# utiasSTARS/pyslam

Measured on AMD Instinct MI355X. Metric: ms/LM-iter (Jac build + J^T J + Schur solve), stereo BA @ 500k residuals, lower is better.
Workload: dtype f64

## Files before the change

pyslam_amd/csrc/ps_abi_problem.h:

```cpp


const char* ps_last_error(void) { return g_err.c_str(); }

int ps_device_count(void) {
    int n = 0;
    if (hipGetDeviceCount(&n) != hipSuccess) return 0;
    return n;
}

int ps_warm_up(void) {
    static std::once_flag once;
    static int rc = 0;
    std::call_once(once, [] {
        void* p = nullptr;
        if (hipMalloc(&p, 256) != hipSuccess) { rc = fail("hipMalloc failed (no usable HIP device?)"); return; }
        hipLaunchKernelGGL(k_zero4, dim3(1), dim3(256), 0, 0, (size_t)8, (double*)p, (size_t)0, (double*)nullptr, (size_t)0,
                           (double*)nullptr, (size_t)0, (double*)nullptr);
        double hostw[4] = {0, 0, 0, 0};
        (void)hipMemsetAsync(p, 0, 256, 0);
        (void)hipMemcpyAsync((char*)p + 128, p, 64, hipMemcpyDeviceToDevice, 0);
        (void)hipMemcpyAsync(hostw, p, sizeof(hostw), hipMemcpyDeviceToHost, 0);
        if (hipDeviceSynchronize() != hipSuccess) rc = fail("the warm-up launch failed");
        hipFree(p);
        hipFuncAttributes a;
// ... 769 lines not shown
        } else {
            int32_t init[2] = {0, INT_MAX}, *d_mm = nullptr;
            if (h->alloc(&d_mm, 2, true)) return -1;
            HIP_OK(hipMemcpyAsync(d_mm, init, sizeof(init), hipMemcpyHostToDevice, h->stream));
            hipLaunchKernelGGL(k_lmw_maxobs, dim3(cdiv(nv, 256)), dim3(256), 0, h->stream, nv, h->lm_ptr, d_mm);
            HIP_OK(hipMemcpyAsync(init, d_mm, sizeof(init), hipMemcpyDeviceToHost, h->stream));
            HIP_OK(hipStreamSynchronize(h->stream));
            mx = init[0]; mn = init[1];
        }
        if (mx <= PS_LMW_MAXOBS && mn >= 1) {
            const int W = 64 - (mx - 1), nw = cdiv(Nl, W);
            if (!dev_build) {
                std::vector<int32_t> first((size_t)nw + 1, nv);
                for (int w = 0, v = 0; w < nw; ++w) { while (v < nv && lm_ptr[v] < W * w) ++v; first[w] = v; }
                if (h->upload(&h->lmw_first, first)) return -1;
            } else {
                if (h->alloc(&h->lmw_first, (size_t)nw + 1, true)) return -1;
                hipLaunchKernelGGL(k_lmw_items, dim3(cdiv(nw + 1, 256)), dim3(256), 0, h->stream, nv, nw, W, h->lm_ptr, h->lmw_first);
            }
            h->lmw_nwaves = nw;
            h->nsq_l = std::max(h->nsq_l, cdiv(nw, 4));
        }
    }
    h->nsq_p = nr > 0 ? cdiv(P, 256) : 0;
    if (h->alloc(&h->sq_part_l, (size_t)h->nsq_l) || h->alloc(&h->sq_part_p, (size_t)h->nsq_p) ||
        h->alloc(&h->shard_buf, 2)) return -1;
    if (h->alloc(&h->cost_partials, (size_t)std::max({h->ncost_obs + h->ncost_fac, cdiv(h->lmw_nwaves, 4) + h->ncost_fac, 512}) + 8)) return -1;
    if (h->zero(h->shard_buf, 2 * sizeof(double))) return -1;
    if (!ps_pool().take(ps_pool().host_words, &h->words_host))
        HIP_OK(hipHostMalloc(&h->words_host, PS_WORDS_BYTES, hipHostMallocMapped | hipHostMallocCoherent));
    std::memset(h->words_host, 0, PS_WORDS_BYTES);
    char* wdev = nullptr;
    HIP_OK(hipHostGetDevicePointer((void**)&wdev, h->words_host, 0));
    static_assert(SC_NWORDS * sizeof(double) <= 256 && ST_NWORDS * sizeof(int32_t) <= 256, "result words outgrew their windows");
    char* whost = (char*)h->words_host;
    h->h_scalars = (double*)(whost + 0);      h->h_scalars_dev = (double*)(wdev + 0);
    h->h_status = (int32_t*)(whost + 256);    h->h_status_dev = (int32_t*)(wdev + 256);
    h->h_seq = (long long*)(whost + 512);     h->h_seq_dev = (long long*)(wdev + 512);
    h->h_shard = (double*)(whost + 768);      h->h_shard_dev = (double*)(wdev + 768);
    h->h_setup = (long long*)(whost + 1024);  h->h_setup_dev = (long long*)(wdev + 1024);
    h->h_ldi_fro = (double*)(whost + 1280);   h->h_ldi_fro_dev = (double*)(wdev + 1280);
    h->h_early = (long long*)(whost + 1536);  h->h_early_dev = (long long*)(wdev + 1536);
    h->h_lmfail = (long long*)(whost + 1792); h->h_lmfail_dev = (long long*)(wdev + 1792);
    h->h_mo_hist = (double*)(whost + 2048);   h->h_mo_hist_dev = (double*)(wdev + 2048);
    if (h->alloc(&h->arrivals, 2)) return -1;
    if (h->zero(h->arrivals, 2 * sizeof(int32_t))) return -1;
    if (h->arena_close()) return -1;
    HIP_OK(hipStreamSynchronize(h->stream));
    if (nr >= 16 && nr * D > h->direct_max && h->pcg_variant == 1 && !ps_env("PS_LAZY_COARSE")) {
        if (build_coarse(h)) return -1;
        HIP_OK(hipStreamSynchronize(h->stream));
        lap("two-level structures");
    }
    if (ldi_eligible(h) && h->ldi_direct_ok && h->N == 0 && h->F > 0 && !h->ldi_stream &&
        !ps_pool().take(ps_pool().side_streams, &h->ldi_stream))
        HIP_OK(hipStreamCreateWithFlags(&h->ldi_stream, hipStreamNonBlocking));
    lap("scalars + final sync");
    relook_launch_gates(h);
    guard.ok = true;
    *out = h;
    return 0;
}

int ps_problem_create(const ps_problem_desc* d_in, void* stream, ps_problem** out) {
    return problem_create(d_in, nullptr, stream, out);
}

int ps_problem_create_hybrid(const ps_problem_desc* d_in, const ps_host_rows_desc* rows, void* stream, ps_problem** out) {
    if (!rows) return fail("null argument");
    return problem_create(d_in, rows, stream, out);
}

int ps_set_host_rows(ps_problem* h, const double* rows, int64_t num, double cost) {
    if (!h) return fail("null argument");
    if (!h->hybrid) return fail("ps_set_host_rows: the handle has no host rows (ps_problem_create_hybrid)");
    if (num != h->FH) return fail("ps_set_host_rows: row count differs from the create call's");
    if (num > 0 && !rows) return fail("null argument");
    const size_t FROW = 3 * (size_t)h->D * h->D + 2 * (size_t)h->D;
    if (num > 0) {
        HIP_OK(hipMemcpyAsync(h->fscratch + (size_t)h->F * FROW, rows, (size_t)num * FROW * sizeof(double), hipMemcpyHostToDevice, h->stream));
        HIP_OK(hipStreamSynchronize(h->stream));
    }
    h->host_cost = cost;
    h->prelin_valid = false;
    h->last_cost = h->prev_cost = -1.0;
    return 0;
}
```

pyslam_amd/csrc/ps_abi_solver.h:

```cpp

int ps_get_info(ps_problem* h, ps_problem_info* info) {
    if (!h || !info) return fail("null argument");
    info->dof = h->D; info->num_poses = h->P; info->num_reduced = h->nr; info->num_points = h->L;
    info->num_var_points = h->nv; info->num_obs = h->N; info->num_edges = h->F; info->num_priors = 0;
    info->reduced_nnzb = h->nnzb; info->num_pairs = h->npairs;
    info->reduce_count = ((long)h->nnzb + h->nr) / 2 * h->D * h->D + (long)h->nr * h->D + 3;
    info->device_bytes = (int64_t)h->dev_bytes;
    info->cg_restarts = h->cg_fallbacks;
    info->cg_kernel_launches = h->cg_kernel_launches;
    info->ldi_solves = h->ldi_solves; info->ldi_fallbacks = h->ldi_fallbacks; info->ldi_seeds = h->ldi_seeds;
    info->xcg_fused_solves = h->xf_solves; info->xcg_fused_fallbacks = h->xf_fallbacks;
    info->cg_persist_solves = h->cp_launches; info->cg_persist_failures = h->cp_failures;
    info->cg_persist_refused = h->cp_refused; info->persist_cus = h->persist_cus;
    info->persist_cus_needed = h->cp_ok ? h->cp_cus_needed : (h->xp_ok ? h->xp_cus_needed : 0);
    info->landmark_passes_taken_over = h->prelm_used;
    return 0;
}

int ps_eval_cost(ps_problem* h, int include_all_constant, double* cost) {
    if (!h || !cost) return fail("null argument");
    if (include_all_constant && h->fuse_cost == 1 && lm_cost_possible(h)) { if (lm_cost_pass(h, h->lin_lambda, SC_COST)) return -1; }
    else if (cost_pass(h, include_all_constant, SC_COST)) return -1;
    if (read_scalars(h)) return -1;
    *cost = h->h_scalars[SC_COST];
    if (include_all_constant && !h->hybrid) h->last_cost = *cost;
    return 0;
}

int ps_linearize(ps_problem* h, double lambda) {
    if (!h) return fail("null argument");
    h->last_cost = h->prev_cost = -1.0;
    return linearize(h, lambda);
}

static int ensure_shard_pack(ps_problem* h) {
    if (h->shard_pack) return 0;
    const int nr = h->nr, DD = h->D * h->D;
    std::vector<int32_t> up, upT;
    for (int r = 0; r < nr; ++r)
        for (int b = h->h_row_ptr[r]; b < h->h_row_ptr[r + 1]; ++b) {
            const int c = h->h_col_idx[b];
            if (c < r) continue;
            up.push_back(b);
            const int32_t* lo = h->h_col_idx.data() + h->h_row_ptr[c];
            const int32_t* hi = h->h_col_idx.data() + h->h_row_ptr[c + 1];
            const int32_t* it = std::lower_bound(lo, hi, r);
            if (it == hi || *it != r) return fail("reduced block pattern is not symmetric");
            upT.push_back((int32_t)(it - h->h_col_idx.data()));
        }
    h->nup = (long)up.size();
    h->pack_count = h->nup * DD + (long)nr * h->D + 2 + 1;
    if (h->upload(&h->up_slot, up) || h->upload(&h->upT_slot, upT) || h->alloc(&h->shard_pack, (size_t)h->pack_count)) return -1;
    relook_launch_gates(h);
    return 0;
}

int ps_reduce_buffer(ps_problem* h, void** dev_ptr, int64_t* count) {
    if (!h || !dev_ptr || !count) return fail("null argument");
    if (ensure_shard_pack(h)) return -1;
    *dev_ptr = h->shard_pack; *count = h->pack_count;
    return 0;
}

int ps_shard_pack(ps_problem* h) {
    if (!h) return fail("null argument");
    if (ensure_shard_pack(h)) return -1;
    const long ntail = (long)h->nr * h->D + 2;
    const int nb = (int)std::min<long>(4096, cdiv(h->pack_count, 256));
    if (h->D == 6) hipLaunchKernelGGL(k_shard_pack<6>, dim3(nb), dim3(256), 0, h->stream, h->nup, h->up_slot, h->S, ntail, h->g, h->status, h->shard_pack);
    else hipLaunchKernelGGL(k_shard_pack<3>, dim3(nb), dim3(256), 0, h->stream, h->nup, h->up_slot, h->S, ntail, h->g, h->status, h->shard_pack);
    return 0;
}

int ps_shard_unpack(ps_problem* h) {
    if (!h) return fail("null argument");
    h->prelin_valid = h->prelm_valid = false;
    if (ensure_shard_pack(h)) return -1;
    const long ntail = (long)h->nr * h->D + 2;
    const int nb = (int)std::min<long>(4096, cdiv(h->pack_count, 256));
    if (h->D == 6) hipLaunchKernelGGL(k_shard_unpack<6>, dim3(nb), dim3(256), 0, h->stream, h->nup, h->up_slot, h->upT_slot, h->shard_pack, h->S, ntail, h->g, h->status);
    else hipLaunchKernelGGL(k_shard_unpack<3>, dim3(nb), dim3(256), 0, h->stream, h->nup, h->up_slot, h->upT_slot, h->shard_pack, h->S, ntail, h->g, h->status);
    return 0;
}

static inline double resolve_pcg_tol(const ps_problem* h, double tol) {
    if (tol > 0.0) return tol;
    return h->nv > 0 ? 1e-12 : 1e-14;
}

int ps_solve_reduced(ps_problem* h, double tol, int max_iters, int* iters_out, double* relres_out) {
    if (!h) return fail("null argument");
    tol = resolve_pcg_tol(h, tol);
    const int rc = solve_reduced(h, tol, max_iters, iters_out, relres_out);
    if (rc == 0 && h->h_status[ST_LM_FAIL]) return fail("a landmark block H_ll is not positive definite");
    return rc;
}

static int z_of_last_linearize(ps_problem* h, const char* who) {
    if (!h->z_foreign || h->nv == 0) return 0;
    char buf[320];
    snprintf(buf, sizeof buf, "%s: Z, C^-1 and c no longer belong to the last ps_linearize -- a landmark pass has since run at another point "
             "(ps_eval_cost after the parameters moved, or a whole-iteration call that expected a successor): call ps_linearize again", who);
    return fail(buf);
}

int ps_backsub(ps_problem* h) {
    if (!h) return fail("null argument");
    if (z_of_last_linearize(h, "ps_backsub")) return -1;
    return backsub(h);
}

int ps_get_dx(ps_problem* h, double* dx_pose, double* dx_point) {
    if (!h) return fail("null argument");
    std::vector<double> tmp;
    if (dx_pose && h->nr) HIP_OK(hipMemcpyAsync(dx_pose, h->x, (size_t)h->nr * h->D * sizeof(double), hipMemcpyDefault, h->stream));
    if (dx_point && h->nv) {
        tmp.resize((size_t)h->nv * 3);
        HIP_OK(hipMemcpyAsync(tmp.data(), h->dxl, tmp.size() * sizeof(double), hipMemcpyDeviceToHost, h->stream));
    }
    if (sync(h)) return -1;
    for (int s2 = 0; dx_point && s2 < h->nv; ++s2)
        std::memcpy(dx_point + 3 * (size_t)h->h_vid_of_slot[s2], &tmp[3 * (size_t)s2], 3 * sizeof(double));
    return 0;
}

int ps_step_norm2(ps_problem* h, double* norm2) {
    if (!h || !norm2) return fail("null argument");
    if (step_norm(h) || read_scalars(h)) return -1;
    *norm2 = h->h_scalars[SC_DXP2] + h->h_scalars[SC_DXL2];
    return 0;
}

int ps_apply_update(ps_problem* h, double step) {
    if (!h) return fail("null argument");
    h->prelin_valid = h->prelm_valid = false;
    h->last_cost = h->prev_cost = -1.0;
    return apply_update(h, step);
}

int ps_snapshot_params(ps_problem* h) {
    if (!h) return fail("null argument");
    h->snap_valid = true;
    h->snap_cost = h->last_cost;
    const size_t n1 = (size_t)h->P * h->PW, n2 = (size_t)h->L * 3;
    if (n1 + n2)
        hipLaunchKernelGGL(k_copy2, dim3((unsigned)std::min<size_t>(2048, cdiv((long)(n1 + n2), 256))), dim3(256), 0, h->stream,
                           n1, (const double*)h->poses, h->poses_snap, n2, (const double*)h->points, h->points_snap);
    return 0;
}

static int restore_params_by_exchange(ps_problem* h) {
    if (!h->snap_valid) return fail("ps_solve: no snapshot to restore");
    h->params_moved_since_lin = true;
    h->prelin_valid = h->prelm_valid = false;
    h->last_cost = h->snap_cost; h->prev_cost = -1.0;
    std::swap(h->poses, h->poses_snap);
    std::swap(h->points, h->points_snap);
    h->snap_valid = false;
    return 0;
}

int ps_restore_params(ps_problem* h) {
    if (!h) return fail("null argument");
    if (!h->snap_valid) return fail("ps_restore_params: no snapshot (none taken, or ps_solve has consumed it)");
    h->params_moved_since_lin = true;
    h->prelin_valid = h->prelm_valid = false;
    h->last_cost = h->snap_cost; h->prev_cost = -1.0;
    const size_t n1 = (size_t)h->P * h->PW, n2 = (size_t)h->L * 3;
    if (n1 + n2)
        hipLaunchKernelGGL(k_copy2, dim3((unsigned)std::min<size_t>(2048, cdiv((long)(n1 + n2), 256))), dim3(256), 0, h->stream,
                           n1, (const double*)h->poses_snap, h->poses, n2, (const double*)h->points_snap, h->points);
    return 0;
}

int ps_get_params(ps_problem* h, double* poses, double* points) {
    if (!h) return fail("null argument");
    if (poses && h->P) HIP_OK(hipMemcpyAsync(poses, h->poses, (size_t)h->P * h->PW * sizeof(double), hipMemcpyDefault, h->stream));
    if (points && h->L) HIP_OK(hipMemcpyAsync(points, h->points, (size_t)h->L * 3 * sizeof(double), hipMemcpyDefault, h->stream));
    return sync(h);
}

int ps_set_params(ps_problem* h, const double* poses, const double* points) {
    if (!h) return fail("null argument");
    h->params_moved_since_lin = true;
    h->prelin_valid = h->prelm_valid = false;
    h->last_cost = h->prev_cost = -1.0;
    if (poses && h->P) HIP_OK(hipMemcpyAsync(h->poses, poses, (size_t)h->P * h->PW * sizeof(double), hipMemcpyDefault, h->stream));
    if (points && h->L) HIP_OK(hipMemcpyAsync(h->points, points, (size_t)h->L * 3 * sizeof(double), hipMemcpyDefault, h->stream));
    return sync(h);
}

int ps_gn_finish(ps_problem* h, int linesearch, double* cost_out, double* dx_pose_norm2, double* dx_point_norm2) {
    if (!h) return fail("null argument");
    if (z_of_last_linearize(h, "ps_gn_finish")) return -1;
    HIP_OK(hipMemsetAsync(h->scalars + SC_DXP2, 0, sizeof(double), h->stream));
    HIP_OK(hipMemsetAsync(h->scalars + SC_DXL2, 0, sizeof(double), h->stream));
    if (gn_tail(h, linesearch, nullptr)) return -1;
    if (read_scalars(h)) return -1;
    if (h->h_status[ST_LM_FAIL]) return fail("a landmark block H_ll is not positive definite");
    if (cost_out) *cost_out = linesearch ? h->h_scalars[SC_COST] : h->h_scalars[SC_LINCOST];
    if (dx_pose_norm2) *dx_pose_norm2 = h->h_scalars[SC_DXP2];
    if (dx_point_norm2) *dx_point_norm2 = h->h_scalars[SC_DXL2];
    return 0;
}

int ps_gn_solve_finish(ps_problem* h, double pcg_tol, int pcg_max_iters, int linesearch, double* cost_out,
                       double* dx_pose_norm2, double* dx_point_norm2, int* pcg_iters_out, double* pcg_relres_out) {
    if (!h) return fail("null argument");
    pcg_tol = resolve_pcg_tol(h, pcg_tol);
    if (z_of_last_linearize(h, "ps_gn_solve_finish")) return -1;
    HIP_OK(hipMemsetAsync(h->scalars + SC_DXP2, 0, sizeof(double), h->stream));
    HIP_OK(hipMemsetAsync(h->scalars + SC_DXL2, 0, sizeof(double), h->stream));
    if (h->nr > 0 && h->pcg_variant == 1) {
        const int rc = h->D == 6
            ? gn_solve_and_finish_async<6>(h, pcg_tol, pcg_max_iters, linesearch, pcg_iters_out, pcg_relres_out, nullptr)
            : gn_solve_and_finish_async<3>(h, pcg_tol, pcg_max_iters, linesearch, pcg_iters_out, pcg_relres_out, nullptr);
        if (rc) return -1;
    } else {
        if (solve_reduced(h, pcg_tol, pcg_max_iters, pcg_iters_out, pcg_relres_out)) return -1;
        if (gn_tail(h, linesearch, nullptr)) return -1;
        if (read_scalars(h)) return -1;
    }
    if (h->h_status[ST_LM_FAIL]) return fail("a landmark block H_ll is not positive definite");
    if (cost_out) *cost_out = linesearch ? h->h_scalars[SC_COST] : h->h_scalars[SC_LINCOST];
    if (dx_pose_norm2) *dx_pose_norm2 = h->h_scalars[SC_DXP2];
    if (dx_point_norm2) *dx_point_norm2 = h->h_scalars[SC_DXL2];
    return 0;
}

int ps_set_segment_exchange(ps_problem* h, void* nccl_all_gather_fn, int32_t world, int32_t rank, int64_t maxlen,
                            int64_t n_mine, const int64_t* mine, int64_t n_dst, const int64_t* dst, const int64_t* src_ptr,
                            const int64_t* src_off) {
    if (!h) return fail("null argument");
    if (!nccl_all_gather_fn) { h->seg_allgather = nullptr; return 0; }
    if (!(h->nccl_allreduce && h->nccl_comm)) return fail("ps_set_segment_exchange: call ps_set_collective first");
    if (ensure_shard_pack(h)) return -1;
    const int64_t T = 3, body = h->pack_count - T;
    if (world < 1 || rank < 0 || rank >= world || n_mine < 0 || n_dst < 0 || maxlen < T + n_mine || (n_mine && !mine) ||
        (n_dst && (!dst || !src_ptr || !src_off)))
        return fail("ps_set_segment_exchange: inconsistent plan");
    for (int64_t k = 0; k < n_mine; ++k) if (mine[k] < 0 || mine[k] >= body) return fail("ps_set_segment_exchange: an element of this rank lies outside [upper(S) | g]");
    for (int64_t k = 0; k < n_dst; ++k) {
        if (dst[k] < 0 || dst[k] >= body || src_ptr[k + 1] < src_ptr[k]) return fail("ps_set_segment_exchange: bad destination table");
        for (int64_t q = src_ptr[k]; q < src_ptr[k + 1]; ++q) {
            const int64_t r = src_off[q] / maxlen, o = src_off[q] % maxlen;
            if (src_off[q] < 0 || r >= world || o < T || (q > src_ptr[k] && src_off[q] / maxlen <= src_off[q - 1] / maxlen))
                return fail("ps_set_segment_exchange: bad source table (offsets must be rank * maxlen + 3 + k, ascending rank)");
        }
    }
    if (n_dst && src_ptr[0] != 0) return fail("ps_set_segment_exchange: src_ptr must start at 0");
    if ((int64_t)world * maxlen > INT32_MAX || body > INT32_MAX) return fail("ps_set_segment_exchange: the exchange does not fit 32-bit plan entries");
    const std::vector<int32_t> vm(mine, mine + n_mine), vd(dst, dst + n_dst), vp(src_ptr, src_ptr + (n_dst ? n_dst + 1 : 0)),
                               vo(src_off, src_off + (n_dst ? src_ptr[n_dst] : 0));
    if (h->upload(&h->seg_mine, vm) || h->upload(&h->seg_dst, vd) || h->upload(&h->seg_src_ptr, vp) || h->upload(&h->seg_src_off, vo) ||
        h->alloc(&h->seg_in, (size_t)maxlen) || h->alloc(&h->seg_all, (size_t)maxlen * world)) return -1;
    h->seg_world = world; h->seg_maxlen = maxlen; h->seg_nmine = n_mine; h->seg_ndst = n_dst;
    h->seg_allgather = (ps_problem::allgather_fn)nccl_all_gather_fn;
    return 0;
}

static int exchange_reduced_system(ps_problem* h) {
    enum { NCCL_F64 = 8, NCCL_SUM = 0 };
    if (!h->seg_allgather) {
        { StageTimer tpk(h, PS_ST_PACK); if (ps_shard_pack(h)) return -1; }
        {
            StageTimer tar(h, PS_ST_ALLREDUCE);
            if (h->nccl_allreduce(h->shard_pack, h->shard_pack, (size_t)h->pack_count, NCCL_F64, NCCL_SUM, h->nccl_comm, h->stream))
                return fail("ncclAllReduce of the reduced system failed");
        }
        { StageTimer tpk(h, PS_ST_PACK); if (ps_shard_unpack(h)) return -1; }
        return 0;
    }
    h->prelin_valid = h->prelm_valid = false;
    const long T = 3, ntail = (long)h->nr * h->D + 2;
    const unsigned nb1 = (unsigned)std::min<long>(2048, cdiv(h->seg_maxlen, 256)), nb2 = (unsigned)std::min<long>(4096, cdiv(h->seg_ndst + T, 256));
    {
        StageTimer tpk(h, PS_ST_PACK);
        if (h->D == 6) hipLaunchKernelGGL(k_seg_pack<6>, dim3(nb1), dim3(256), 0, h->stream, h->nup, h->up_slot, h->S, ntail, h->g, h->status, T, h->seg_nmine, h->seg_mine, h->seg_in, h->seg_maxlen);
        else hipLaunchKernelGGL(k_seg_pack<3>, dim3(nb1), dim3(256), 0, h->stream, h->nup, h->up_slot, h->S, ntail, h->g, h->status, T, h->seg_nmine, h->seg_mine, h->seg_in, h->seg_maxlen);
    }
    {
        StageTimer tar(h, PS_ST_ALLREDUCE);
        if (h->seg_allgather(h->seg_in, h->seg_all, (size_t)h->seg_maxlen, NCCL_F64, h->nccl_comm, h->stream))
            return fail("ncclAllGather of the reduced system's segments failed");
    }
    {
        StageTimer tpk(h, PS_ST_PACK);
        if (h->D == 6) hipLaunchKernelGGL(k_seg_sum<6>, dim3(nb2), dim3(256), 0, h->stream, h->seg_ndst, h->seg_dst, h->seg_src_ptr, h->seg_src_off, h->seg_all, T, h->seg_world, h->seg_maxlen, h->nup, h->up_slot, h->upT_slot, h->S, ntail, h->g, h->status);
        else hipLaunchKernelGGL(k_seg_sum<3>, dim3(nb2), dim3(256), 0, h->stream, h->seg_ndst, h->seg_dst, h->seg_src_ptr, h->seg_src_off, h->seg_all, T, h->seg_world, h->seg_maxlen, h->nup, h->up_slot, h->upT_slot, h->S, ntail, h->g, h->status);
    }
    return 0;
}

int ps_set_collective(ps_problem* h, void* nccl_all_reduce_fn, void* nccl_comm) {
    if (!h) return fail("null argument");
    if (h->hybrid && nccl_comm) return fail("a hybrid handle (host rows) is not landmark-sharded");
    h->nccl_allreduce = (ps_problem::allreduce_fn)nccl_all_reduce_fn;
    h->nccl_comm = nccl_comm;
    relook_launch_gates(h);
    return 0;
}

int ps_shard_buffer(ps_problem* h, void** dev_ptr) {
    if (!h || !dev_ptr) return fail("null argument");
    *dev_ptr = h->shard_buf;
    return 0;
}

int ps_gn_solve_finish_enqueue(ps_problem* h, double pcg_tol, int pcg_max_iters, int linesearch, int first) {
    if (!h) return fail("null argument");
    if (h->nr == 0 || h->pcg_variant != 1) return fail("ps_gn_solve_finish_enqueue needs the fused CG and a reduced system");
    pcg_tol = resolve_pcg_tol(h, pcg_tol);
    if (first && z_of_last_linearize(h, "ps_gn_solve_finish_enqueue")) return -1;
    h->shard_out = true;
    h->no_repeat = !(h->nccl_allreduce && h->nccl_comm);
    struct Reset { ps_problem* h; ~Reset() { h->shard_out = false; h->no_repeat = false; } } reset{h};
    if (first) {
        HIP_OK(hipMemsetAsync(h->scalars + SC_DXP2, 0, sizeof(double), h->stream));
        if (!h->coarse_built && build_coarse(h)) return -1;
        if (!(h->nccl_allreduce && h->nccl_comm) && h->xf_skip == 0) h->xf_skip = 1;
        if (h->cg_explicit) { if (h->D == 6 ? xcg_setup<6>(h, pcg_max_iters, true) : xcg_setup<3>(h, pcg_max_iters, true)) return -1; }
        else if (h->D == 6 ? cg_fused_setup<6>(h, pcg_max_iters, true) : cg_fused_setup<3>(h, pcg_max_iters, true)) return -1;
    }
    const int limit = pcg_max_iters + (h->cg_explicit ? 1 : 2);
    const bool big_step = h->prev_cost > 0.0 && h->last_cost > 0.0 && std::fabs(h->prev_cost - h->last_cost) > 0.05 * h->prev_cost;
    const int margin = big_step ? (h->cg_explicit ? 5 : std::max(6, h->cg_margin))
                                : ((h->cg_explicit || h->last_pcg_iters == h->prev_pcg_iters) ? std::min(2, h->cg_margin) : h->cg_margin);
    int count = first ? (h->last_pcg_iters > 0 ? h->last_pcg_iters + margin : (h->cg_explicit ? 32 : 24)) : std::max(8, h->cg_launched / 2);
    count = std::min(count, limit - h->cg_launched);
    const bool last = count <= 0;
    const int32_t* gate = last ? nullptr : h->status;
    if (h->cg_explicit) {
        if (!last) {
            const int head = std::min(count, 12);
            if (h->D == 6) { xcg_launch<6>(h, pcg_tol, head); if (xcg_side_enqueue<6>(h)) return -1; xcg_launch<6>(h, pcg_tol, count - head); }
            else { xcg_launch<3>(h, pcg_tol, head); if (xcg_side_enqueue<3>(h)) return -1; xcg_launch<3>(h, pcg_tol, count - head); }
        }
        if (h->D == 6) hipLaunchKernelGGL(k_cg_unscale<6>, dim3(cdiv((long)h->nr * 6, 256)), dim3(256), 0, h->stream, h->nr, h->Linv, h->cg_xh, h->x, gate);
        else hipLaunchKernelGGL(k_cg_unscale<3>, dim3(cdiv((long)h->nr * 3, 256)), dim3(256), 0, h->stream, h->nr, h->Linv, h->cg_xh, h->x, gate);
    } else if (h->D == 6) { if (!last) cg_fused_launch<6>(h, pcg_tol, count); cg_fused_recover<6>(h, gate); }
    else { if (!last) cg_fused_launch<3>(h, pcg_tol, count); cg_fused_recover<3>(h, gate); }
    if (gn_tail(h, linesearch, last ? nullptr : h->status)) return -1;
    return last ? 1 : 0;
}

int ps_gn_result(ps_problem* h, int* done, double* shard2 , double* dx_pose_norm2,
                 int* pcg_iters_out, double* pcg_relres_out) {
    if (!h) return fail("null argument");
    double sb[2] = {0.0, 0.0};
    HIP_OK(hipMemcpyAsync(sb, h->shard_buf, sizeof(sb), hipMemcpyDeviceToHost, h->stream));
    if (read_scalars(h)) return -1;
    if (h->h_status[ST_LM_FAIL]) return fail("a landmark block H_ll is not positive definite");
    if (done) *done = h->h_status[ST_PCG_DONE];
    if (shard2) { shard2[0] = sb[0]; shard2[1] = sb[1]; }
    if (dx_pose_norm2) *dx_pose_norm2 = h->h_scalars[SC_DXP2];
    if (h->h_status[ST_PCG_DONE]) { h->prev_cost = h->last_cost; h->last_cost = sb[0]; }
// ... 195 lines not shown

static int lm_iteration_impl(ps_problem* h, double lambda, double pcg_tol, int pcg_max_iters, int linesearch, double* cost_out,
                             double* dx_norm_out, double* model_decrease_out, int* pcg_iters_out, double* pcg_relres_out,
                             double* start_cost_out) {
    if (!h) return fail("null argument");
    if (h->nccl_allreduce && h->nccl_comm) return fail("ps_lm_iteration: not offered for a landmark-sharded handle");
    if (!linesearch) return fail("ps_lm_iteration: the gain ratio needs the cost AFTER the step (linesearch != 0)");
    if (!(lambda >= 0.0) || !std::isfinite(lambda)) return fail("ps_lm_iteration: lambda must be finite and >= 0");
    const int expect_was = h->expect_next;
    const bool spec_was = h->spec_next;
    h->expect_next = 0; h->spec_next = false;
    h->lm_md = true;
    const int rc = gn_iteration_impl(h, lambda, pcg_tol, pcg_max_iters, linesearch, cost_out, dx_norm_out, pcg_iters_out, pcg_relres_out,
                                     start_cost_out);
    h->lm_md = false;
    h->expect_next = expect_was; h->spec_next = spec_was;
    if (rc) return rc;
    if (model_decrease_out) *model_decrease_out = h->h_scalars[SC_MODELDEC];
    return 0;
}

int ps_lm_iteration(ps_problem* h, double lambda, double pcg_tol, int pcg_max_iters, int linesearch, double* cost_out,
                    double* dx_norm_out, double* model_decrease_out, int* pcg_iters_out, double* pcg_relres_out) {
    return lm_iteration_impl(h, lambda, pcg_tol, pcg_max_iters, linesearch, cost_out, dx_norm_out, model_decrease_out, pcg_iters_out,
                             pcg_relres_out, nullptr);
}

int ps_solve_lm(ps_problem* h, const ps_lm_options* o, double pcg_tol, int pcg_max_iters, double* cost_history, int32_t cap,
                int32_t* n_history, int32_t* iterations, double* last_dx_norm, int32_t* pcg_iters, double* pcg_relres, double* iter_ms,
                double* lm_rows) {
    if (!h || !o || !cost_history || !n_history) return fail("null argument");
    if (h->nccl_allreduce && h->nccl_comm) return 1;
    if (h->hybrid) return 1;
    if (o->max_iters < 0 || (long)o->max_iters + 2 > cap) return 1;
    if (!(o->lambda_min > 0.0) || !(o->lambda_max >= o->lambda_min)) return fail("ps_solve_lm: 0 < lambda_min <= lambda_max expected");
    if (ps_reset_solver_state(h)) return -1;
    auto clamp = [&](double v) { return std::min(std::max(v, o->lambda_min), o->lambda_max); };
    double lam = clamp(o->lambda0 > 0.0 ? o->lambda0 : 1e-3), nu = 2.0;
    int n = 0, it = 0;
    double cost = 0.0, dxn = 0.0;
    bool done = false;
    while (!done) {
        ++it;
        h->solve_horizon = -1;
        if (ps_snapshot_params(h)) return -1;
        const auto t0 = std::chrono::steady_clock::now();
        double c0 = 0.0, c = 0.0, rel = 0.0, md = 0.0;
        int its = 0;
        if (lm_iteration_impl(h, lam, pcg_tol, pcg_max_iters, o->linesearch, &c, &dxn, &md, &its, &rel, it == 1 ? &c0 : nullptr)) return -1;
        if (it == 1) { cost = c0; cost_history[n++] = c0; }
        const double prev = cost;
        const bool ok = std::isfinite(md) && md > 0.0 && std::isfinite(c);
        const double rho = ok ? (prev - c) / md : -1.0;
        const double used = lam, raw = lam * nu;
        const bool accepted = rho > 0.0;
        if (accepted) {
            const double q = 2.0 * rho - 1.0;
            cost = c; lam = clamp(lam * std::max(1.0 / 3.0, 1.0 - q * q * q)); nu = 2.0;
        } else {
            lam = clamp(raw); nu *= 2.0;
            if (restore_params_by_exchange(h)) return -1;
            h->last_cost = prev;
        }
        if (lm_rows) { double* r = lm_rows + 4 * (size_t)(it - 1); r[0] = used; r[1] = rho; r[2] = accepted ? 1.0 : 0.0; r[3] = md; }
        if (pcg_iters) pcg_iters[it - 1] = its;
        if (pcg_relres) pcg_relres[it - 1] = rel;
        if (iter_ms) iter_ms[it - 1] = std::chrono::duration<double, std::milli>(std::chrono::steady_clock::now() - t0).count();
        cost_history[n++] = cost;
        static_assert(offsetof(ps_lm_options, lambda0) == sizeof(ps_solve_options), "ps_lm_options begins with ps_solve_options' fields");
        done = ps_stop_base(reinterpret_cast<const ps_solve_options*>(o), it, cost, dxn);
        if (accepted) done = done || cost >= o->min_cost_decrease * prev;
        else done = done || raw > o->lambda_max;
    }
    h->snap_valid = false;
    *n_history = n;
    if (iterations) *iterations = it;
    if (last_dx_norm) *last_dx_norm = dxn;
    return 0;
}

int ps_motion_only_solve(ps_problem* h, const ps_solve_options* o, double* cost_history, int32_t cap, int32_t* n_history,
                         int32_t* iterations, double* last_dx_norm, double* pose12_out) {
    if (!h || !o || !cost_history || !n_history) return fail("null argument");
    h->prelin_valid = h->prelm_valid = false;
    const bool eligible = h->mo_fused && !h->hybrid && h->nv == 0 && h->F == 0 && h->nr == 1 && h->P == 1 && h->D == 6 && h->N == h->Np &&
                          h->pcg_variant == 1 && h->max_pose_obs <= 2048;
    const int need = o->max_iters + 2;
    if (!eligible || need + 16 > PS_MO_HIST_WORDS || need > cap) return 1;
    h->cov_ready = false;
    h->last_cost = h->prev_cost = -1.0;
    if (!h->status_clean) {
        HIP_OK(hipMemsetAsync(h->status, 0, ST_NWORDS * sizeof(int32_t), h->stream));
        h->status_clean = true;
    }
    const ObsWide wp{h->sidx_p, h->stiff_tab};
    const long long seq_now = ++h->seq;
    StageTimer total(h, PS_ST_TOTAL, 2);
    if (h->wide_obs)
        hipLaunchKernelGGL(k_motion_only_solve<true>, dim3(1), dim3(PS_MO_THREADS), 0, h->stream, h->pitems, h->pitem_ptr, h->pobs,
                           h->points, h->ogroups, h->poses, *o, h->x, h->status, h->scalars, h->h_mo_hist_dev, PS_MO_HIST_WORDS,
                           h->h_status_dev, h->h_scalars_dev, h->h_seq_dev, seq_now, wp);
    else
        hipLaunchKernelGGL(k_motion_only_solve<false>, dim3(1), dim3(PS_MO_THREADS), 0, h->stream, h->pitems, h->pitem_ptr, h->pobs,
                           h->points, h->ogroups, h->poses, *o, h->x, h->status, h->scalars, h->h_mo_hist_dev, PS_MO_HIST_WORDS,
                           h->h_status_dev, h->h_scalars_dev, h->h_seq_dev, seq_now, wp);
    total.stop();
    if (wait_published(h)) return -1;
    if (h->h_status[ST_DIAG_FAIL]) {
        h->status_clean = false;
        return fail("reduced system has a non-positive-definite diagonal block (gauge freedom? hold a pose constant or add a prior)");
    }
    const int n = (int)h->h_mo_hist[0];
    if (n < 1 || n > cap) return fail("ps_motion_only_solve: cost history out of range");
    for (int k = 0; k < n; ++k) cost_history[k] = h->h_mo_hist[15 + k];
    if (pose12_out) for (int k = 0; k < 12; ++k) pose12_out[k] = h->h_mo_hist[3 + k];
    *n_history = n;
    if (iterations) *iterations = (int32_t)h->h_mo_hist[1];
    if (last_dx_norm) *last_dx_norm = h->h_mo_hist[2];
    h->last_cost = cost_history[n - 1];
    return 0;
}

int ps_covariance_begin(ps_problem* h) {
    if (!h) return fail("null argument");
    cov_release(h);
    ++h->cov_epoch;
    h->prelin_valid = h->prelm_valid = false;
    if (linearize(h, 0.0)) return -1;
    if (h->nr > 0 && h->pcg_variant == 1 && !use_direct(h) && !h->coarse_built && build_coarse(h)) return -1;
    if (h->nr > 0 && h->pcg_variant == 1 && !use_direct(h) && !h->cg_explicit) {
        const int rc = h->D == 6 ? cg_fused_setup<6>(h, 16) : cg_fused_setup<3>(h, 16);
        if (rc) return -1;
    }
    if (read_scalars(h)) return -1;
    if (h->h_status[ST_LM_FAIL]) return fail("a landmark block H_ll is not positive definite");
    if (h->h_status[ST_DIAG_FAIL]) return fail("reduced system has a non-positive-definite diagonal block (gauge freedom? hold a pose constant or add a prior)");
    if (h->h_slot_of_vid.size() != h->h_vid_of_slot.size()) {
        h->h_slot_of_vid.assign(h->h_vid_of_slot.size(), 0);
        for (size_t s2 = 0; s2 < h->h_vid_of_slot.size(); ++s2) h->h_slot_of_vid[h->h_vid_of_slot[s2]] = (int32_t)s2;
    }
    h->cov_ready = true;
    return 0;
}

int ps_covariance_column(ps_problem* h, int kind, int index, int comp, double tol, int max_iters,
                         int* iters_out, double* relres_out) {
    if (!h) return fail("null argument");
    tol = resolve_pcg_tol(h, tol);
    if (!h->cov_ready) return fail("ps_covariance_column: call ps_covariance_begin first (any linearisation invalidates it)");
    if (kind == 0 ? (index < 0 || index >= h->nr || comp < 0 || comp >= h->D)
                  : (kind != 1 || index < 0 || index >= h->nv || comp < 0 || comp >= 3))
        return fail("ps_covariance_column: parameter index / component out of range");
    if (h->nr) HIP_OK(hipMemsetAsync(h->g, 0, (size_t)h->nr * h->D * sizeof(double), h->stream));
    if (h->nv) HIP_OK(hipMemsetAsync(h->cvec, 0, (size_t)h->nv * 3 * sizeof(double), h->stream));
    const int slot = kind == 1 ? h->h_slot_of_vid[index] : index;
    hipLaunchKernelGGL(k_cov_rhs, dim3(1), dim3(64), 0, h->stream, kind, slot, comp, h->D, h->lm_ptr, h->lobs,
                       h->pose_rid, h->Z, h->Cinv, h->g, h->cvec);
    int its = 0; double rel = 0.0;
    if (h->nr > 0) {
        int rc;
        if (use_direct(h)) {
            rc = h->D == 6 ? direct_solve_enqueue<6>(h) : direct_solve_enqueue<3>(h);
            if (!rc) rc = read_scalars(h);
            if (!rc) rc = cg_report(h, &its, &rel);
        } else if (h->pcg_variant == 1 && h->cg_explicit)
            rc = h->D == 6 ? xcg_run<6>(h, tol, max_iters, &its, &rel) : xcg_run<3>(h, tol, max_iters, &its, &rel);
        else if (h->pcg_variant == 1)
            rc = h->D == 6 ? cg_fused_run<6>(h, tol, max_iters, &its, &rel, true) : cg_fused_run<3>(h, tol, max_iters, &its, &rel, true);
        else
            rc = h->D == 6 ? pcg_run<6>(h, tol, max_iters, &its, &rel) : pcg_run<3>(h, tol, max_iters, &its, &rel);
        if (rc) return -1;
    }
    if (backsub(h)) return -1;
    if (iters_out) *iters_out = its;
    if (relres_out) *relres_out = rel;
    return 0;
}

int ps_get_reduced_system(ps_problem* h, int32_t* row_ptr, int32_t* col_idx, double* vals, double* g) {
    if (!h) return fail("null argument");
    if (row_ptr) std::memcpy(row_ptr, h->h_row_ptr.data(), h->h_row_ptr.size() * sizeof(int32_t));
    if (col_idx) std::memcpy(col_idx, h->h_col_idx.data(), h->h_col_idx.size() * sizeof(int32_t));
    if (vals && h->nnzb) HIP_OK(hipMemcpyAsync(vals, h->S, (size_t)h->nnzb * h->D * h->D * sizeof(double), hipMemcpyDeviceToHost, h->stream));
    if (g && h->nr) HIP_OK(hipMemcpyAsync(g, h->g, (size_t)h->nr * h->D * sizeof(double), hipMemcpyDeviceToHost, h->stream));
    return sync(h);
}

int ps_get_landmark_factors(ps_problem* h, double* cinv, double* c) {
    if (!h) return fail("null argument");
    if (z_of_last_linearize(h, "ps_get_landmark_factors")) return -1;
    std::vector<double> t6((size_t)h->nv * 6), t3((size_t)h->nv * 3);
    if (h->nv) {
        HIP_OK(hipMemcpyAsync(t6.data(), h->Cinv, t6.size() * sizeof(double), hipMemcpyDeviceToHost, h->stream));
        HIP_OK(hipMemcpyAsync(t3.data(), h->cvec, t3.size() * sizeof(double), hipMemcpyDeviceToHost, h->stream));
    }
    if (sync(h)) return -1;
    for (int s2 = 0; s2 < h->nv; ++s2) {
        const size_t v = (size_t)h->h_vid_of_slot[s2];
        if (cinv) std::memcpy(cinv + 6 * v, &t6[6 * (size_t)s2], 6 * sizeof(double));
        if (c) std::memcpy(c + 3 * v, &t3[3 * (size_t)s2], 3 * sizeof(double));
    }
    return 0;
}

int ps_debug_reproj_blocks(ps_problem* h, double* r, double* jpose, double* jpoint) {
    if (!h || !r || !jpose || !jpoint) return fail("null argument");
    if (h->N == 0) return 0;
    double *dr, *djp, *djl;
    HIP_OK(hipMalloc((void**)&dr, (size_t)h->N * 3 * sizeof(double)));
    HIP_OK(hipMalloc((void**)&djp, (size_t)h->N * 18 * sizeof(double)));
    HIP_OK(hipMalloc((void**)&djl, (size_t)h->N * 9 * sizeof(double)));
    const ObsWide wl{h->sidx_l, h->stiff_tab};
    if (h->wide_obs)
        hipLaunchKernelGGL(k_debug_reproj<true>, dim3(cdiv(h->N, 256)), dim3(256), 0, h->stream, h->N, h->lobs, h->lorig,
                       h->poses, h->points, h->ogroups, dr, djp, djl, wl);
    else
        hipLaunchKernelGGL(k_debug_reproj<false>, dim3(cdiv(h->N, 256)), dim3(256), 0, h->stream, h->N, h->lobs, h->lorig,
                       h->poses, h->points, h->ogroups, dr, djp, djl, wl);
    hipMemcpyAsync(r, dr, (size_t)h->N * 3 * sizeof(double), hipMemcpyDeviceToHost, h->stream);
    hipMemcpyAsync(jpose, djp, (size_t)h->N * 18 * sizeof(double), hipMemcpyDeviceToHost, h->stream);
    hipMemcpyAsync(jpoint, djl, (size_t)h->N * 9 * sizeof(double), hipMemcpyDeviceToHost, h->stream);
    const int rc = sync(h);
    hipFree(dr); hipFree(djp); hipFree(djl);
    return rc;
}

int ps_debug_factor_blocks(ps_problem* h, double* r, double* j1, double* j2) {
    if (!h || !r || !j1 || !j2) return fail("null argument");
    if (h->F == 0) return 0;
    const int D = h->D, DD = D * D, ROW = D + 2 * DD;
    double* dbg;
    HIP_OK(hipMalloc((void**)&dbg, (size_t)h->F * ROW * sizeof(double)));
    const int rc0 = D == 6 ? launch_factor_pass<6>(h, 0.0, dbg) : launch_factor_pass<3>(h, 0.0, dbg);
    std::vector<double> t((size_t)h->F * ROW);
    hipMemcpyAsync(t.data(), dbg, t.size() * sizeof(double), hipMemcpyDeviceToHost, h->stream);
    const int rc = sync(h);
    hipFree(dbg);
    if (rc0 || rc) return -1;
    for (long f = 0; f < h->F; ++f) {
        std::memcpy(r + f * D, &t[(size_t)f * ROW], D * sizeof(double));
        std::memcpy(j1 + f * DD, &t[(size_t)f * ROW + D], DD * sizeof(double));
        std::memcpy(j2 + f * DD, &t[(size_t)f * ROW + D + DD], DD * sizeof(double));
    }
    return 0;
}

int ps_debug_table_checksums(ps_problem* h, uint64_t* out, int capacity, int* count) {
    if (!h || !out || !count) return fail("null argument");
    if (sync(h)) return -1;
    struct Tab { const void* p; size_t bytes; };
    const bool tiled = h->schur_tiles > 1 && h->npair_items > 0;
    const Tab tabs[16] = {
        {h->point_vid, (size_t)h->L * 4}, {h->lobs, (size_t)h->N * sizeof(LObs)}, {h->lorig, (size_t)h->N * 4},
        {h->lm_ptr, ((size_t)h->nv + 1) * 4}, {h->lm_point, (size_t)h->nv * 4}, {h->pose_of_rid, (size_t)std::max(h->nr, 1) * 4},
        {h->pitems, (size_t)h->npitems * sizeof(PItem)}, {h->pitem_ptr, ((size_t)h->nr + 1) * 4}, {h->pobs, (size_t)h->Np * sizeof(LObs)},
        {h->pairs, (size_t)h->npairs * 8}, {h->pair_xitems, (size_t)8 * h->pair_per_xcd * sizeof(PairItem)},
        {tiled ? h->comb_items : nullptr, (size_t)h->ncomb * sizeof(PairItem)}, {tiled ? h->comb_tasks : nullptr, (size_t)h->npair_items * 4},
        {h->row_ptr, ((size_t)h->nr + 1) * 4}, {h->col_idx, (size_t)h->nnzb * 4}, {h->diag_slot, (size_t)h->nr * 4}};
    *count = 16;
    std::vector<unsigned char> buf;
    for (int t = 0; t < 16 && t < capacity; ++t) {
        uint64_t hsh = 0;
        if (tabs[t].p && tabs[t].bytes) {
            buf.resize(tabs[t].bytes);
            HIP_OK(hipMemcpy(buf.data(), tabs[t].p, tabs[t].bytes, hipMemcpyDeviceToHost));
            hsh = 1469598103934665603ull;
            size_t i = 0;
            for (; i + 8 <= buf.size(); i += 8) { uint64_t w; std::memcpy(&w, &buf[i], 8); hsh = (hsh ^ w) * 1099511628211ull; }
            for (; i < buf.size(); ++i) hsh = (hsh ^ buf[i]) * 1099511628211ull;
        }
        out[t] = hsh;
    }
    return 0;
}

static void relook_path(ps_problem* h) {
    const bool possible = ps_ldi_possible(*h, (long)h->nr * h->D);
    if (h->coarse_built && possible != h->xmin_auto_ldi && h->cg_explicit_min_rows < 0) h->coarse_built = false;
}

int ps_set_option(ps_problem* h, const char* name, double value) {
    if (!h || !name) return fail("null argument");
    if (!std::strcmp(name, "expect_next")) { h->expect_next = value != 0 && !h->hybrid; return 0; }
    if (!std::strcmp(name, "solve_horizon")) { h->solve_horizon = value < 0 ? -1 : (int)std::min(value, 1e6); return 0; }
    h->prelin_valid = h->prelm_valid = false;
    const char* refusal = nullptr;
    const int fx = ps_option_apply(*h, name, value, &refusal);
    if (fx == PS_OPT_UNKNOWN) return fail(std::string("unknown option: ") + name);
    if (fx == PS_OPT_REFUSED) return fail(refusal);
    if (fx & PS_FX_COARSE_REBUILD) h->coarse_built = false;
    if (fx & PS_FX_DROP_FACTOR) h->lci_next = -1;
    if (fx & PS_FX_DROP_SIDE) h->side_todo = false;
    if ((fx & PS_FX_LDI_OFF) && !h->ldi_enable) { h->ldi_cur = -1; if (h->ldi_state != 1) h->ldi_state = 0; }
    if (fx & PS_FX_RELOOK_PATH) relook_path(h);
    relook_launch_gates(h);
    return 0;
}

int ps_get_option(ps_problem* h, const char* name, double* value) {
    if (!h || !name || !value) return fail("null argument");
    const std::string n(name);
    if (n == "lin_zero_list") *value = h->lin_zero_gate ? 1.0 : 0.0;
    else if (n == "lin_fills") *value = (double)h->lin_fills;
    else if (n == "lin_zero_launches") *value = (double)h->lin_zero_launches;
    else return fail("ps_get_option: no read-back for option: " + n);
    return 0;
}

int ps_reset_solver_state(ps_problem* h) {
    if (!h) return fail("null argument");
    h->prelin_valid = h->prelm_valid = false;
    if (!h->solver_touched) {
        static_cast<PsCostHistory&>(*h) = PsCostHistory{};
        return 0;
    }
    h->solver_touched = false;
    HIP_OK(hipStreamSynchronize(h->stream));
    if (h->side) HIP_OK(hipStreamSynchronize(h->side));
    if (h->ldi_stream) HIP_OK(hipStreamSynchronize(h->ldi_stream));
    drain_timers(h);
    static_cast<PsCarried&>(*h) = PsCarried{};
    static_cast<PsCostHistory&>(*h) = PsCostHistory{};
    if (h->lag_status) HIP_OK(hipMemsetAsync(h->lag_status, 0, ST_NWORDS * sizeof(int32_t), h->stream));
    if (h->ldi_ready && !(h->ldi_direct_ok && h->N == 0 && h->F > 0)) h->ldi_direct = false;
    h->cov_ready = false;
    return 0;
}

#ifndef PS_BUILD_SHA
#define PS_BUILD_SHA "unknown"
#endif
const char* ps_build_sha(void) { return PS_BUILD_SHA; }

int ps_set_profiling(ps_problem* h, int enabled) {
    if (!h) return fail("null argument");
    h->profiling = enabled < 0 ? 0 : (enabled > 2 ? 2 : enabled);
    return 0;
}

int ps_get_stage_times(ps_problem* h, double* ms, int64_t* counts, int reset) {
    if (!h) return fail("null argument");
    if (!h->pending.empty() && sync(h)) return -1;
    for (int i = 0; i < PS_NUM_STAGES; ++i) {
        if (ms) ms[i] = h->stage_ms[i];
        if (counts) counts[i] = h->stage_n[i];
        if (reset) { h->stage_ms[i] = 0.0; h->stage_n[i] = 0; }
    }
    return 0;
}

int ps_dense_normal_solve(const double* J, const double* r, int32_t m, int32_t n, double* dx, double* covariance) {
    if (!J || !r || !dx || m <= 0 || n <= 0) return fail("bad argument");
    if (n > 2048) return fail("generic (host-evaluated) path supports at most 2048 unknowns");
    int ndev = 0;
    if (hipGetDeviceCount(&ndev) != hipSuccess || ndev == 0) return fail("no HIP device visible");
    const int nrhs = covariance ? n + 1 : 1;
    DevBuf bJ, br, bH, bB, bst, bg;
    if (bJ.get((size_t)m * n * sizeof(double)) || br.get((size_t)m * sizeof(double)) || bH.get((size_t)n * n * sizeof(double)) ||
        bB.get((size_t)n * nrhs * sizeof(double)) || bst.get(ST_NWORDS * sizeof(int32_t)) || bg.get((size_t)n * sizeof(double))) return -1;
    double *dJ = bJ.as<double>(), *dr = br.as<double>(), *dH = bH.as<double>(), *dB = bB.as<double>(), *dg = bg.as<double>();
    int32_t* dst = bst.as<int32_t>();
    HIP_OK(hipMemset(dst, 0, ST_NWORDS * sizeof(int32_t)));
    HIP_OK(hipMemcpy(dJ, J, (size_t)m * n * sizeof(double), hipMemcpyHostToDevice));
    HIP_OK(hipMemcpy(dr, r, (size_t)m * sizeof(double), hipMemcpyHostToDevice));
    hipLaunchKernelGGL(k_dense_normal, dim3(cdiv((long)n * n, 256)), dim3(256), 0, 0, m, n, dJ, dr, dH, dg);
    std::vector<double> B((size_t)n * nrhs, 0.0), gh(n);
    HIP_OK(hipMemcpy(gh.data(), dg, (size_t)n * sizeof(double), hipMemcpyDeviceToHost));
    for (int i = 0; i < n; ++i) { B[(size_t)i * nrhs] = gh[i]; if (covariance) B[(size_t)i * nrhs + 1 + i] = 1.0; }
    HIP_OK(hipMemcpy(dB, B.data(), B.size() * sizeof(double), hipMemcpyHostToDevice));
    hipLaunchKernelGGL(k_dense_chol_solve, dim3(1), dim3(256), 0, 0, n, nrhs, dH, dB, dst);
    HIP_OK(hipMemcpy(B.data(), dB, B.size() * sizeof(double), hipMemcpyDeviceToHost));
    int32_t st[ST_NWORDS];
    HIP_OK(hipMemcpy(st, dst, sizeof(st), hipMemcpyDeviceToHost));
    for (int i = 0; i < n; ++i) {
        dx[i] = B[(size_t)i * nrhs];
        if (covariance) for (int j = 0; j < n; ++j) covariance[(size_t)i * n + j] = B[(size_t)i * nrhs + 1 + j];
    }
    if (st[ST_DIAG_FAIL]) return fail("normal matrix is not positive definite");
    return 0;
}
```

pyslam_amd/csrc/ps_abi_triang.h:

```cpp

int ps_triangulate(ps_problem* h, int64_t n, const int32_t* vids, int refine_iters, double min_parallax_deg, int write_back,
                   double* points_out, int32_t* status_out) {
    if (!h) return fail("null argument");
    if (h->nv > 0 && h->D != 6) return fail("ps_triangulate: landmarks on a problem whose poses are not SE(3)");
    if (refine_iters < 0 || refine_iters > 1000) return fail("ps_triangulate: refine_iters must lie in [0, 1000]");
    if (!(min_parallax_deg >= 0.0 && min_parallax_deg <= 180.0)) return fail("ps_triangulate: min_parallax_deg must lie in [0, 180]");
    if (!vids) n = h->nv;
    if (n < 0) return fail("ps_triangulate: negative count");
    if (n == 0) return 0;
    if (n >= (1L << 31) / 16) return fail("ps_triangulate: too many landmarks for one call");
    if (h->h_slot_of_vid.size() != h->h_vid_of_slot.size()) {
        h->h_slot_of_vid.assign(h->h_vid_of_slot.size(), 0);
        for (size_t s2 = 0; s2 < h->h_vid_of_slot.size(); ++s2) h->h_slot_of_vid[h->h_vid_of_slot[s2]] = (int32_t)s2;
    }
    std::vector<int32_t> slots;
    if (vids) {
        slots.resize((size_t)n);
        for (int64_t k = 0; k < n; ++k) {
            if (vids[k] < 0 || vids[k] >= h->nv)
                return fail("ps_triangulate: landmark index " + std::to_string(vids[k]) + " out of range (variable landmarks: " +
                            std::to_string(h->nv) + ")");
            slots[k] = h->h_slot_of_vid[vids[k]];
        }
    }
    const size_t words = (size_t)n * 3 + (size_t)n;
    if (h->tri_cap < words) {
        if (h->tri_buf) { hipStreamSynchronize(h->stream); hipFree(h->tri_buf); h->tri_buf = nullptr; h->tri_cap = 0; }
        void* p = nullptr;
        const hipError_t e = hipMalloc(&p, words * sizeof(double));
        if (e != hipSuccess) return fail(std::string("ps_triangulate: hipMalloc: ") + hipGetErrorString(e));
        h->tri_buf = (double*)p; h->tri_cap = words;
    }
    double* d_pts = h->tri_buf;
    int32_t* d_status = reinterpret_cast<int32_t*>(h->tri_buf + (size_t)n * 3);
    int32_t* d_slots = d_status + n;
    hipStream_t st = h->stream;
    if (vids) HIP_OK(hipMemcpyAsync(d_slots, slots.data(), (size_t)n * sizeof(int32_t), hipMemcpyHostToDevice, st));
    const double cos_min = std::cos(min_parallax_deg * (3.14159265358979323846 / 180.0));
    const ObsWide wl{h->sidx_l, h->stiff_tab};
    const dim3 grid(cdiv(n, 256 / PS_LM_GROUP)), block(256);
    if (h->wide_obs)
        hipLaunchKernelGGL(k_triangulate<true>, grid, block, 0, st, (int)n, vids ? d_slots : (const int32_t*)nullptr, h->lm_ptr, h->lm_point,
                           h->lobs, h->poses, h->points, h->ogroups, wl, refine_iters, cos_min, write_back ? 1 : 0, d_pts, d_status);
    else
        hipLaunchKernelGGL(k_triangulate<false>, grid, block, 0, st, (int)n, vids ? d_slots : (const int32_t*)nullptr, h->lm_ptr, h->lm_point,
                           h->lobs, h->poses, h->points, h->ogroups, wl, refine_iters, cos_min, write_back ? 1 : 0, d_pts, d_status);
    if (write_back) {
        h->params_moved_since_lin = true;
        h->prelin_valid = h->prelm_valid = false;
        h->last_cost = h->prev_cost = -1.0;
    }
    std::vector<double> pts(points_out && !vids ? (size_t)n * 3 : 0);
    std::vector<int32_t> stat(status_out && !vids ? (size_t)n : 0);
    if (points_out) HIP_OK(hipMemcpyAsync(vids ? points_out : pts.data(), d_pts, (size_t)n * 3 * sizeof(double), hipMemcpyDeviceToHost, st));
    if (status_out) HIP_OK(hipMemcpyAsync(vids ? status_out : stat.data(), d_status, (size_t)n * sizeof(int32_t), hipMemcpyDeviceToHost, st));
    if (sync(h)) return -1;
    if (!vids)
        for (int64_t s2 = 0; s2 < n; ++s2) {
            const int32_t vid = h->h_vid_of_slot[s2];
            if (points_out) std::memcpy(points_out + 3 * (size_t)vid, &pts[3 * (size_t)s2], 3 * sizeof(double));
            if (status_out) status_out[vid] = stat[s2];
        }
    return 0;
}
```

pyslam_amd/csrc/ps_core.hip:

```cpp
#include <hip/hip_runtime.h>

#include <algorithm>
#include <array>
#include <map>
#include <atomic>
#include <chrono>
#include <thread>
#include <climits>
#include <cmath>
#include <cstdio>
#include <cstring>
#include <memory>
#include <mutex>
#include <string>
#include <vector>

#include "pyslam_hip.h"
#include "ps_kernels.h"
#include "ps_ransac.h"
#include "ps_k_twoview.h"
#include "ps_k_pnp.h"
#include "ps_photo.h"
#include "ps_k_dense.h"
#include "ps_k_feat.h"
// ... 120 lines not shown
    double xcg_tag_lambda[2] = {0.0, 0.0}, xcg_setup_lambda = 0.0;
    bool mc_active = false;
    bool last_setup_lagx = false;
    int xf_skip = 0;
    int ldi_state = 0;
    int ldi_cur = -1, ldi_next = -1;
    long ldi_iter = 0, ldi_ready_at = 0;
    bool ldi_side_todo = false, ldi_update_ok = false, ldi_sread_pending = false;
    int ldi_last_its = 0, ldi_prev_its = 0;
    int ldi_rejects = 0; long ldi_no_seed_before = 0;
    double ldi_tag = -1.0, ldi_next_tag = -1.0, ldi_call_start_cost = -1.0;
    double ldi_prev_start_cost = -2.0;
    bool ldi_moved = false;
    int last_pcg_iters = 0;
    int prev_pcg_iters = -1;
};

struct ps_problem : PsOptions, PsCostHistory, PsCarried {
    hipStream_t stream = nullptr;
    bool own_stream = false;
    int D = 6, PW = 12;
    int P = 0, nr = 0, L = 0, nv = 0;
    long N = 0, Nl = 0, Np = 0;
    long F = 0;
    long FH = 0;
    bool hybrid = false;
    double host_cost = 0.0;
    long npairs = 0;
    int nnzb = 0;
    size_t dev_bytes = 0;
    std::vector<void*> allocs;
    struct Guard { char* guard; size_t table_bytes; int serial; };
    std::vector<Guard> guards;
    int check_guards(const char* where) {
        int bad = 0;
        std::vector<unsigned char> g(4096);
        for (const Guard& gd : guards) {
            if (hipMemcpy(g.data(), gd.guard, 4096, hipMemcpyDeviceToHost) != hipSuccess) return -1;
            for (int i = 0; i < 4096; ++i) if (g[i] != 0xA5) {
                fprintf(stderr, "GUARD %p %s: table #%d (%zu bytes) overrun at +%d (byte %02x)\n", (void*)this, where, gd.serial, gd.table_bytes, i, g[i]);
                ++bad; break;
            }
        }
        return bad;
    }

    double *poses = nullptr, *points = nullptr, *poses_snap = nullptr, *points_snap = nullptr;
    int32_t *pose_rid = nullptr, *point_vid = nullptr;
    ObsGroup* ogroups = nullptr;
    bool wide_obs = false;
    int32_t *sidx_l = nullptr, *sidx_p = nullptr;
    double* stiff_tab = nullptr;
    LObs* lobs = nullptr;
    int32_t *lorig = nullptr, *lm_ptr = nullptr, *lm_point = nullptr;
    double *Z = nullptr, *Cinv = nullptr, *cvec = nullptr, *dxl = nullptr;
    LObs* pobs = nullptr;
    PItem* pitems = nullptr;
    int npitems = 0;
    int32_t* pitem_ptr = nullptr;
    double* ppartial = nullptr;
    int2* pairs = nullptr;
    int npair_items = 0, pair_per_xcd = 0;
    PairItem* pair_xitems = nullptr;
    int schur_tiles = 1, ncomb = 0;
    bool has_diag_tasks = false;
    double* Spart = nullptr;
    PairItem* comb_items = nullptr;
    int32_t* comb_tasks = nullptr;
    FactorGroup* fgroups = nullptr;
    int32_t *f_i = nullptr, *f_j = nullptr, *f_grp = nullptr;
    double *f_Tinv = nullptr, *fscratch = nullptr;
    int32_t *eslots = nullptr, *eptr = nullptr, *eslot_diag = nullptr, *gptr = nullptr, *gitems = nullptr;
    int2* eitems = nullptr;
    int nes = 0;
    int32_t *row_ptr = nullptr, *col_idx = nullptr, *diag_slot = nullptr;
    double* red = nullptr;
    long red_count = 0;
    double *S = nullptr, *g = nullptr;
    int32_t* zero_slots = nullptr;
    int nzero_slots = 0;
    bool has_extra_pairs = false;
    bool lin_zero_gate = false;
    long lin_fills = 0, lin_zero_launches = 0;
    std::vector<int32_t> h_row_ptr, h_col_idx;
    std::vector<int32_t> h_vid_of_slot;
    double *x = nullptr, *r = nullptr, *z = nullptr, *p0 = nullptr, *p1 = nullptr, *q = nullptr, *Minv = nullptr;
    double *rz_part = nullptr, *rr_part = nullptr, *pq_part = nullptr, *hist = nullptr;
    int npartA = 0, npartB = 0, hist_cap = 0;
    double *Linv = nullptr, *cg_r[2] = {}, *cg_w[2] = {}, *cg_s[2] = {}, *cg_gd[2] = {}, *cg_xh = nullptr;
    int32_t* brow_of = nullptr;
    double* cg_p = nullptr;
    double* Saug = nullptr;
    int32_t* ident_slot = nullptr;
    int G = 0, ncb = 0, nc = 0, nr_aug = 0, nnzb_aug = 0;
    size_t cg_cap = 0, saug_cap = 0;
    int32_t *pnode = nullptr, *slo = nullptr, *shi = nullptr, *run_lo = nullptr, *run_hi = nullptr,
            *arow_ptr = nullptr, *acol_idx = nullptr, *aug_slot = nullptr, *fine_nnz = nullptr;
    double *pw0 = nullptr, *pw1 = nullptr, *SZ = nullptr, *Ac = nullptr, *tvec = nullptr, *chol_scratch = nullptr;
    double *Bmat = nullptr, *bgv = nullptr, *SB = nullptr, *BSZ = nullptr;
    double *Bmat2[2] = {}, *X2[2] = {}, *Mpart = nullptr;
    bool lagx_ok = false;
    int side_buf = 0;
    double host_wait_ns = 0.0, host_call_ns = 0.0;
    long host_waits = 0, host_calls = 0;
    size_t rows_lds = 0;
    bool rows_attr_set = false, rows_lci_lds = false;
    int32_t *ent_ptr = nullptr, *ent_q = nullptr, *ent_lo = nullptr, *ent_hi = nullptr;
    int32_t *seg_ptr = nullptr, *seg_ent = nullptr, *seg_row = nullptr;
    int max_row_ents = 0;
    int32_t* pose_of_rid = nullptr;
    double *Lci2[2] = {}, *LciT2[2] = {};
    hipStream_t side = nullptr;
    int side_cus = 0;
    hipEvent_t ev_ac = nullptr, ev_chol = nullptr, ev_acdone = nullptr;
    unsigned long long* chk_sums = nullptr; int chk_nsum = 0;
    double *chk_Ac = nullptr, *chk_BSZ = nullptr, *chk_Ac_side = nullptr; int32_t* chk_cnt = nullptr; size_t chk_bsz_n = 0;
    int32_t* lag_status = nullptr;
    double* Mc = nullptr;
    bool coarse_built = false;
    bool coarse_clamped = false;
    int max_pose_obs = 0;
    double* mo_partials = nullptr;
    bool status_clean = true;
    double *dA = nullptr, *dLi = nullptr, *dLiT = nullptr;
    bool cg_explicit = false;
    double lin_lambda = 0.0;
    double *xstate = nullptr, *xy = nullptr, *xp2 = nullptr;
    int ac_bw = -1;
    std::unique_ptr<BandPart> bpart;
    double *Lrow = nullptr, *Lcol = nullptr, *rdiag = nullptr;
    bool xcg_rt_ok = false;
    int xcg_rt_rows = PS_XCG_ROWS_RT;
    int32_t *xcg_wg_out = nullptr, *xcg_nptr = nullptr;
    double *tq_part = nullptr, *tvec2 = nullptr;
    bool xf_ok = false, xf_active = false;
    bool xf_one_ok = false, xf_two = false;
    int32_t *xf_cptr = nullptr, *xf_cols = nullptr, *xf_nlo = nullptr, *xf_nhi = nullptr, *xf_rec = nullptr;
    uint16_t* xf_lidx = nullptr;
    double *xf_tq[2] = {}, *xf_ts[2] = {}, *xf_t[2] = {};
    int xf_rmax = 1, xf_nwg = 0, xf_pf = 2;
    size_t xf_nrec = 0;
    long xf_solves = 0, xf_fallbacks = 0;
    bool cp_ok = false;
    bool cp_recovered = false;
    int cp_ntasks = 0, cg_max_launches = 0;
    void* cp_tasks = nullptr;
    int32_t* cp_row_task0 = nullptr;
    unsigned long long* cp_exch = nullptr;
    unsigned cp_salt = 0;
    long cp_launches = 0, cp_failures = 0;
    int persist_dev = 0, persist_cus = 0;
    bool persist_masked = false;
    int cp_cus_needed = 0, xp_cus_needed = 0;
    int persist_held = 0;
    bool params_moved_since_lin = false;
    bool z_foreign = false;
    bool no_repeat = false;
    long cp_refused = 0;
    void persist_release() { if (persist_held) { ps_persist_ledger().release(persist_dev, persist_held); persist_held = 0; } }
    int persist_capacity() const { return persist_masked ? persist_cus / 2 : persist_cus; }
    bool persist_reserve(int need) {
        if (need <= 0 || persist_cus <= 0) return false;
        if (persist_held) return true;
        if (!ps_persist_ledger().reserve(persist_dev, need, persist_capacity())) { ++cp_refused; return false; }
        persist_held = need; return true;
    }
// ... 127 lines not shown
        dev_bytes += bytes;
        *out = (T*)p;
        return 0;
    }
    char* slab = nullptr; size_t slab_left = 0;
    int slab_reserve(size_t bytes) {
        if (ps_env("PS_ALLOC_GUARD")) return 0;
        void* p = nullptr;
        hipError_t e = hipMalloc(&p, bytes);
        if (e != hipSuccess) return fail(std::string("hipMalloc: ") + hipGetErrorString(e));
        if (ps_env("PS_ARENA_POISON") && hipMemset(p, 0xFF, bytes) != hipSuccess) return fail("hipMemset (poison) failed");
        allocs.push_back(p);
        slab = (char*)p; slab_left = bytes;
        return 0;
    }
    void slab_close() { slab = nullptr; slab_left = 0; }
    bool in_arena(const void* p) const {
        return arena_open && (const char*)p >= arena_dev && (const char*)p < arena_dev + PS_ARENA_BYTES;
    }
    template <typename T>
    int upload(T** out, const T* src, size_t n, bool src_resident = false) {
        if (alloc(out, n)) return -1;
        if (!n) return 0;
        if (src_resident) {
            if (in_arena(*out)) HIP_OK(hipMemcpy(arena_host + ((char*)*out - arena_dev), src, n * sizeof(T), hipMemcpyDeviceToHost));
            else HIP_OK(hipMemcpy(*out, src, n * sizeof(T), hipMemcpyDeviceToDevice));
            return 0;
        }
        if (in_arena(*out)) std::memcpy(arena_host + ((char*)*out - arena_dev), src, n * sizeof(T));
        else HIP_OK(hipMemcpy(*out, src, n * sizeof(T), hipMemcpyHostToDevice));
        return 0;
    }
    template <typename T>
    int upload(T** out, const std::vector<T>& v) { return upload(out, v.data(), v.size()); }
    int zero(void* p, size_t bytes) {
        if (in_arena(p)) return 0;
        HIP_OK(hipMemsetAsync(p, 0, std::max<size_t>(bytes, 1), stream));
        return 0;
    }
    int arena_begin() {
        PsPool& pool = ps_pool();
        void *d = nullptr, *m = nullptr;
        if (!pool.take(pool.dev_arenas, &d)) HIP_OK(hipMalloc(&d, PS_ARENA_BYTES));
        arena_dev = (char*)d;
        if (!pool.take(pool.host_arenas, &m)) HIP_OK(hipHostMalloc(&m, PS_ARENA_BYTES, hipHostMallocDefault));
        arena_host = (char*)m;
        static const bool poison = ps_env("PS_ARENA_POISON") != nullptr;
        if (poison) std::memset(arena_host, 0xFF, PS_ARENA_BYTES);
        arena_poisoned = poison;
        arena_used = 0;
        arena_open = true;
        return 0;
    }
    int arena_flush() {
        if (arena_open && arena_used) HIP_OK(hipMemcpyAsync(arena_dev, arena_host, arena_used, hipMemcpyHostToDevice, stream));
        return 0;
    }
    int arena_close() {
        arena_open = false;
        if (arena_poisoned) arena_used = PS_ARENA_BYTES;
        if (arena_used) HIP_OK(hipMemcpyAsync(arena_dev, arena_host, arena_used, hipMemcpyHostToDevice, stream));
        return 0;
    }
    void arena_release() {
        PsPool& pool = ps_pool();
        if (arena_dev && !pool.give(pool.dev_arenas, (void*)arena_dev)) hipFree(arena_dev);
        if (arena_host && !pool.give(pool.host_arenas, (void*)arena_host)) hipHostFree(arena_host);
        if (words_host && !pool.give(pool.host_words, words_host)) hipHostFree(words_host);
        arena_dev = arena_host = nullptr; words_host = nullptr;
    }
};

inline void cov_release(ps_problem* h) {
    if (!h->cov_buf) return;
    hipStreamSynchronize(h->stream);
    hipFree(h->cov_buf);
    h->cov_buf = nullptr;
    h->cov_sigma_epoch = -1;
}

inline void relook_launch_gates(ps_problem* h) {
    const bool shard = (h->nccl_allreduce && h->nccl_comm) || h->seg_allgather || h->shard_pack || h->has_extra_pairs;
    h->lin_zero_gate = h->lin_zero_list && h->zero_slots && !h->Spart && h->schur_pipeline && h->npitems > 0 && h->D == 6 && !shard;
}

#include "ps_host_cg.h"
#include "ps_host_ldi.h"
#include "ps_host_iteration.h"
#include "ps_host_build.h"

extern "C" {

#include "ps_abi_problem.h"
#include "ps_abi_solver.h"
#include "ps_abi_cov.h"
#include "ps_abi_triang.h"
#include "ps_abi_small.h"
#include "ps_abi_twoview.h"
#include "ps_abi_pnp.h"
#include "ps_abi_dense.h"
#include "ps_abi_feat.h"

}
```

pyslam_amd/csrc/ps_host_cg.h:

```cpp

namespace {

struct StageTimer {
    ps_problem* h;
    int stage;
    hipEvent_t a = nullptr, b = nullptr;
    int slot = -1;
    StageTimer(ps_problem* h_, int st, int level = 2) : h(h_), stage(st) {
        if (h->profiling < level) return;
        if (h->profiling == 1 && h->prof_every > 1 &&
            h->prof_tick % h->prof_every != (st == PS_ST_CG_KERNEL ? h->prof_every / 2 : 0)) return;
        if (h->ev_used + 2 > h->ev_pool.size()) {
            for (int i = 0; i < 64; ++i) { hipEvent_t e; hipEventCreate(&e); h->ev_pool.push_back(e); }
        }
        slot = (int)h->ev_used;
        a = h->ev_pool[h->ev_used++];
        b = h->ev_pool[h->ev_used++];
        hipEventRecord(a, h->stream);
    }
    void stop() {
        if (!a) return;
        hipEventRecord(b, h->stream);
        h->pending.push_back({stage, slot});
        a = nullptr;
    }
    ~StageTimer() { stop(); }
};

void drain_timers(ps_problem* h) {
    for (auto& pr : h->pending) {
        float ms = 0.f;
        if (hipEventElapsedTime(&ms, h->ev_pool[pr.second], h->ev_pool[pr.second + 1]) == hipSuccess) {
            h->stage_ms[pr.first] += ms;
            h->stage_n[pr.first] += 1;
        }
    }
    h->pending.clear();
    h->ev_used = 0;
}

int side_kick(ps_problem* h);
int ldi_side_kick(ps_problem* h);
int linearize(ps_problem* h, double lambda, bool allow_prelm = false);

void drain_timers_ready(ps_problem* h) {
    std::vector<std::pair<int, int>> keep;
    for (auto& pr : h->pending) {
        float ms = 0.f;
        if (hipEventQuery(h->ev_pool[pr.second + 1]) != hipSuccess) { keep.push_back(pr); continue; }
        if (hipEventElapsedTime(&ms, h->ev_pool[pr.second], h->ev_pool[pr.second + 1]) == hipSuccess) {
            h->stage_ms[pr.first] += ms;
            h->stage_n[pr.first] += 1;
        }
    }
    h->pending.swap(keep);
    if (h->pending.empty()) h->ev_used = 0;
}

int sync(ps_problem* h) {
    HIP_OK(hipStreamSynchronize(h->stream));
    h->persist_release();
    drain_timers(h);
    if (h->side_todo) h->side_ready = true;
    return 0;
}

int wait_published(ps_problem* h) {
    volatile long long* w = h->h_seq;
    struct WaitClock {
        ps_problem* h; std::chrono::steady_clock::time_point t0 = std::chrono::steady_clock::now();
        ~WaitClock() { h->host_wait_ns += std::chrono::duration<double, std::nano>(std::chrono::steady_clock::now() - t0).count(); ++h->host_waits; }
    } wc{h};
    static const int kick_mode = ps_env("PS_SIDE_KICK") ? atoi(ps_env("PS_SIDE_KICK")) : 2;
    volatile long long* ws = h->h_setup;
    for (long spins = 0; spins < 400000000L; ++spins) {
        if (kick_mode == 2 && h->side_todo && !h->side_ready && *ws == h->setup_seq) { h->side_ready = true; if (side_kick(h)) return -1; }
        if (h->ldi_side_todo && *ws == h->setup_seq) { if (ldi_side_kick(h)) return -1; }
        if (h->early_armed && *reinterpret_cast<volatile long long*>(h->h_early) == h->early_seq) {
            h->early_armed = false; h->spec_enqueued = true;
            if (h->prelm_pending) { h->prelm_pending = false; h->prelm_valid = true; }
            if (linearize(h, h->lin_lambda, true)) return -1;
        }
        if (*w == h->seq) {
            h->persist_release();
            if (h->lmfail_check && *reinterpret_cast<volatile long long*>(h->h_lmfail + (h->lmfail_check & 1)) == h->lmfail_check) h->h_status[ST_LM_FAIL] += 1;
            if (h->h_status[ST_PERSIST_FAIL] && (h->cg_persist || h->xcg_persist)) { h->cg_persist = 0; h->xcg_persist = 0; ++h->cp_failures; }
            if (h->start_cost_pending) {
                h->start_cost_pending = false;
                h->last_cost = h->ldi_call_start_cost = h->h_scalars[SC_STARTCOST];
            }
            if (h->side_todo) { h->side_ready = true; if (kick_mode >= 1 && side_kick(h)) return -1; }
            if (h->ldi_side_todo) { if (h->spec_enqueued) h->ldi_side_todo = false; else if (ldi_side_kick(h)) return -1; }
            h->early_armed = false;
            if (h->pending.empty()) return 0;
            if (h->spec_enqueued) { drain_timers_ready(h); return 0; }
            HIP_OK(hipEventSynchronize(h->ev_pool[h->pending.back().second + 1]));
            drain_timers(h);
            return 0;
        }
        __builtin_ia32_pause();
    }
    return sync(h);
}

int read_scalars(ps_problem* h) {
    HIP_OK(hipMemcpyAsync(h->h_scalars, h->scalars, SC_NWORDS * sizeof(double), hipMemcpyDeviceToHost, h->stream));
    HIP_OK(hipMemcpyAsync(h->h_status, h->status, ST_NWORDS * sizeof(int32_t), hipMemcpyDeviceToHost, h->stream));
    return sync(h);
}

struct PairRec { uint64_t key; int32_t a, b, tile; };

template <int D>
int launch_factor_pass(ps_problem* h, double lambda, double* dbg = nullptr) {
    if (h->F == 0 && h->FH == 0) return 0;
    if (h->F > 0)
        hipLaunchKernelGGL(k_factor_pass<D>, dim3(cdiv(h->F, PS_FP_FACTORS)), dim3(256), 0, h->stream, (int)h->F, h->f_i,
                           h->f_j, h->f_Tinv, h->f_grp, h->fgroups, h->poses, h->fscratch, dbg);
    if (dbg) return 0;
    const long threads = (long)h->nes * D * D + (long)h->nr * D;
    hipLaunchKernelGGL(k_factor_assemble<D>, dim3(cdiv(threads, 256)), dim3(256), 0, h->stream, h->nes,
                       h->eslots, h->eptr, h->eitems, h->eslot_diag, h->nr, h->gptr, h->gitems,
                       h->fscratch, lambda, h->S, h->g);
    return 0;
}

// ... 383 lines not shown
inline void copy_doubles(hipStream_t st, double* dst, const double* src, size_t n) {
    if (!n) return;
    hipLaunchKernelGGL(k_copy2, dim3((unsigned)std::min<size_t>(2048, cdiv((long)n, 256))), dim3(256), 0, st, n, src, dst, (size_t)0,
                       (const double*)nullptr, (double*)nullptr);
}

template <int D>
int coarse_factor(ps_problem* h, hipStream_t st, int buf, int32_t* stat) {
    const int nc = h->nc, ncb = h->ncb;
    if (nc <= 90) {
        const size_t chol_lds = 2 * (size_t)nc * nc * sizeof(double);
        if (ensure_dynamic_lds((const void*)k_coarse_chol<D, true>, (size_t)(chol_lds))) return -1;
        hipLaunchKernelGGL((k_coarse_chol<D, true>), dim3(1), dim3(1024), chol_lds, st, ncb, h->Ac, h->Lci2[buf],
                           h->LciT2[buf], stat, nullptr);
    } else if (h->big_chol) {
        double* A = h->chol_scratch;
        double* Tinv = A + (size_t)nc * nc;
        copy_doubles(st, A, h->Ac, (size_t)nc * nc);
        const int nsteps = cdiv(nc, PS_BC_W);
        for (int s2 = 0; s2 < nsteps; ++s2) {
            const int j0 = s2 * PS_BC_W, w = std::min(PS_BC_W, nc - j0), m = nc - j0 - w;
            hipLaunchKernelGGL(k_bchol_panel, dim3(std::max(1, cdiv((long)m * w, 1024))), dim3(256), 0, st, nc, j0, A,
                               Tinv + (size_t)s2 * PS_BC_W * PS_BC_W, stat);
            if (m > 0) {
                const int nt = cdiv(m, 32);
                hipLaunchKernelGGL(k_bchol_update, dim3(nt * (nt + 1) / 2), dim3(256), 0, st, nc, j0, w, A);
            }
        }
        const bool dense_out = nc > PS_BI_S0 && !h->cg_explicit;
        if (dense_out) {
            HIP_OK(hipMemsetAsync(h->Lci2[buf], 0, (size_t)nc * nc * sizeof(double), st));
            HIP_OK(hipMemsetAsync(h->LciT2[buf], 0, (size_t)nc * nc * sizeof(double), st));
        }
        const size_t inv_lds = ((size_t)PS_BI_S0 + PS_BC_W) * PS_BI_CW * sizeof(double);
        hipLaunchKernelGGL(k_btri_inverse, dim3(cdiv(nc, PS_BI_CW)), dim3(256), inv_lds, st, nc, A, Tinv, h->Lci2[buf], h->LciT2[buf]);
        for (int s2 = PS_BI_S0; s2 < nc; s2 *= 2) {
            const int pairs = cdiv(nc, 2 * s2), nt = cdiv(s2, PS_BM_T);
            for (int stage = 0; stage < 2; ++stage)
                hipLaunchKernelGGL(k_btri_merge, dim3(pairs * nt * nt), dim3(256), 0, st, nc, s2, stage, A, h->Lci2[buf], h->LciT2[buf]);
        }
        if (dense_out)
            hipLaunchKernelGGL(k_btri_clear, dim3(cdiv((long)nc * nc, 256)), dim3(256), 0, st, nc, h->LciT2[buf]);
    } else {
        hipLaunchKernelGGL((k_coarse_chol<D, false>), dim3(1), dim3(1024), 0, st, ncb, h->Ac, h->Lci2[buf],
                           h->LciT2[buf], stat, h->chol_scratch);
    }
    return 0;
}

template <int D>
int xcg_coarse_inverse(ps_problem* h, hipStream_t st, int buf, int32_t* stat) {
    const int nc = h->nc;
    if (h->band_chol && h->ac_bw >= 0 && h->band_part) {
        const int B = std::max(h->ac_bw, 1), m = h->band_part_m > 0 ? h->band_part_m : BandPart::auto_m(h->ncb, B);
        if (BandPart::eligible(h->ncb, B, m)) {
            if (!h->bpart || h->bpart->ncb != h->ncb || h->bpart->B != B || h->bpart->m != m || h->bpart->D != D) {
                if (h->bpart) { HIP_OK(hipStreamSynchronize(st)); if (h->side) HIP_OK(hipStreamSynchronize(h->side)); h->dev_bytes -= h->bpart->bytes; }
                h->bpart.reset(new BandPart());
                if (h->bpart->build(h->ncb, D, B, m, st)) { h->bpart.reset(); return -1; }
                h->dev_bytes += h->bpart->bytes;
            }
            return h->bpart->run<D>(st, h->Ac, nc, (float*)h->LciT2[buf], nc, stat);
        }
    }
    if (h->band_chol && h->ac_bw >= 0) {
        HIP_OK(hipMemsetAsync(h->Lrow, 0, (size_t)nc * PS_BAND_W * sizeof(double), st));
        HIP_OK(hipMemsetAsync(h->Lcol, 0, (size_t)nc * PS_BAND_W * sizeof(double), st));
        hipLaunchKernelGGL(k_band_chol<D>, dim3(1), dim3(256), 0, st, h->ncb, std::max(h->ac_bw, 1), (const double*)h->Ac, h->Lrow, h->Lcol, h->rdiag, stat,
                           nc, (const int2*)nullptr);
        static const bool inv_dot = ps_env("PS_BAND_INV_DOT") != nullptr;
        if (inv_dot)
            hipLaunchKernelGGL(k_band_inverse, dim3(cdiv(nc, 4)), dim3(256), 0, st, nc, h->Lrow, h->Lcol, h->rdiag,
                               h->chol_scratch, (float*)h->LciT2[buf]);
        else
            hipLaunchKernelGGL(k_band_inverse_rl<false>, dim3(cdiv(nc, 4)), dim3(256), 0, st, nc, (const double*)h->Lrow, (const double*)h->Lcol,
                               (const double*)h->rdiag, h->chol_scratch, (float*)h->LciT2[buf], (const BandInvItem*)nullptr, (double*)nullptr, nc);
        return 0;
    }
    if (coarse_factor<D>(h, st, buf, stat)) return -1;
    hipLaunchKernelGGL(k_xcg_ainv, dim3(cdiv(nc, PS_AI_T) * (cdiv(nc, PS_AI_T) + 1) / 2), dim3(256), 0, st, nc, h->Lci2[buf], (float*)h->LciT2[buf], nc);
    return 0;
}

template <int D>
int cg_fused_setup(ps_problem* h, int max_iters, bool allow_lag = false, bool rhs_only = false) {
    const int nr = h->nr, cap = h->hist_cap;
    if (max_iters + 2 > cap) return fail("pcg max_iters exceeds the history buffer (4096)");
    if (!h->coarse_built && build_coarse(h)) return -1;
    h->cg_max_launches = max_iters + 2;
    h->cp_recovered = false;
    h->cg_two_level_reduce = h->nr_aug > 2048 || h->cg_split;
    h->cg_short_rows = (long)h->nnzb_aug <= 24L * h->nr_aug;
    const int G = h->G, rows = h->nr_aug;
    const int32_t* rp = h->arow_ptr;
    const int32_t* ci = h->acol_idx;
    if (rhs_only) {
        hipLaunchKernelGGL(k_cg_prepare<D>, dim3(cdiv((long)nr * D, 256)), dim3(256), 0, h->stream, nr, h->g, h->Linv,
                           h->cg_r[0], h->cg_w[0], h->cg_s[0], h->cg_p, h->cg_xh, h->status,
                           G ? h->Bmat : (const double*)nullptr, h->bgv);
        if (G)
            hipLaunchKernelGGL(k_coarse_rhs<D>, dim3(1), dim3(1024), 0, h->stream, nr, h->ncb, h->slo, h->shi, h->pnode,
                               h->pw0, h->pw1, h->LciT2[h->lci_cur], h->arow_ptr, h->Saug, h->tvec, h->cg_r[0], h->cg_w[0],
                               h->cg_s[0], h->cg_p, h->cg_xh, h->cg_split ? 0 : 2, (const int32_t*)nullptr, h->status,
                               h->bgv);
        h->cg_launched = 0;
        return 0;
    }
    if (h->side_pending) {
        HIP_OK(hipStreamWaitEvent(h->stream, h->ev_chol, 0));
        h->side_pending = false;
    }
    if (G && h->lagx_ok && h->lagx && allow_lag && h->coarse_lag && h->lci_next >= 0) {
        const int ncb = h->ncb, nc = h->nc;
        const int use = h->lci_next, nb = use ^ 1;
        h->lci_cur = use;
        h->Bmat = h->Bmat2[use];
        hipLaunchKernelGGL(k_block_jacobi_factor<D>, dim3(cdiv(nr, 4)), dim3(256), 0, h->stream, nr, h->diag_slot,
                           h->S, h->Linv, h->status, h->g, h->cg_r[0], h->cg_w[0], h->cg_s[0], h->cg_p, h->cg_xh,
                           h->poses, h->pose_of_rid, h->coarse_basis, h->Bmat2[nb], h->bgv);
        if (!h->rows_attr_set) {
            if (ensure_dynamic_lds((const void*)k_rows_setup<D>, (size_t)(h->rows_lds))) return -1;
            h->rows_attr_set = true;
        }
        static const int rs_ablate = ps_env("PS_RS_ABLATE") ? atoi(ps_env("PS_RS_ABLATE")) : 0;
        hipLaunchKernelGGL(k_rows_setup<D>, dim3(nr), dim3(PS_RS_THREADS), h->rows_lds, h->stream, nr, ncb, h->row_ptr, h->col_idx,
                           h->aug_slot, h->S, h->Linv, h->Bmat2[use], h->Bmat2[nb], h->arow_ptr, h->fine_nnz,
                           h->run_lo, h->run_hi, h->pnode, h->pw0, h->pw1, h->LciT2[use], h->X2[use], h->cg_r[0],
                           h->Saug, h->SB, h->Mpart, h->rows_lci_lds ? 1 : 0, rs_ablate);
        hipLaunchKernelGGL(k_coarse_mreduce<D>, dim3(cdiv((long)nc * (nc + 1) * 8, 256)), dim3(256), 0, h->stream, nr, ncb,
                           h->shi, h->Mpart, h->pnode, h->arow_ptr, h->Saug, h->cg_r[0], h->cg_w[0], h->cg_s[0], h->cg_p,
                           h->cg_xh, h->lag_status, h->status, h->h_setup_dev, ++h->setup_seq);
        h->mc_active = false;
        h->side_todo = true; h->side_ready = false; h->side_buf = nb;
        h->cg_launched = 0;
        h->last_setup_lagx = true;
        return 0;
    }
    h->last_setup_lagx = false;
    h->side_todo = false;
    if (G) h->Bmat = h->Bmat2[h->lagx_ok ? h->lci_cur : 0];
    hipLaunchKernelGGL(k_block_jacobi_factor<D>, dim3(cdiv(nr, 4)), dim3(256), 0, h->stream, nr, h->diag_slot,
                       h->S, h->Linv, h->status, h->g, h->cg_r[0], h->cg_w[0], h->cg_s[0], h->cg_p, h->cg_xh,
                       h->poses, h->pose_of_rid, h->coarse_basis, G ? h->Bmat : (double*)nullptr, h->bgv);
    hipLaunchKernelGGL(k_scale_blocks<D>, dim3(h->nnzb), dim3(64), 0, h->stream, nr, h->row_ptr, h->col_idx,
                       h->brow_of, h->Linv, h->S, h->aug_slot, h->Saug, G ? h->Bmat : (const double*)nullptr, h->SB);
    if (G) {
        const int ncb = h->ncb, nc = h->nc;
        if (h->side_pending) {
            HIP_OK(hipStreamWaitEvent(h->stream, h->ev_chol, 0));
            h->side_pending = false;
        }
        hipLaunchKernelGGL(k_coarse_rowsums<D>, dim3(nr), dim3(256), (size_t)(ncb + 1) * D * D * sizeof(double), h->stream,
                           nr, ncb, h->run_lo, h->run_hi, h->acol_idx, h->pnode, h->pw0, h->pw1, h->SB, h->SZ, h->Bmat, h->BSZ);
        hipLaunchKernelGGL(k_coarse_matrix<D>, dim3(cdiv((long)ncb * ncb * D * D, 256)), dim3(256), 0, h->stream,
                           nr, ncb, h->slo, h->shi, h->pnode, h->pw0, h->pw1, h->BSZ, h->Ac);
        auto launch_chol = [&](hipStream_t st, int buf, int32_t* stat) -> int { return coarse_factor<D>(h, st, buf, stat); };
        const bool lag = allow_lag && h->coarse_lag && h->lci_next >= 0 && (!h->cg_split || (long)h->nnzb > 24L * nr) &&
                         !(h->lagx_ok && h->lagx);
        if (lag && h->cg_split && !h->Mc && h->alloc(&h->Mc, (size_t)nc * nc)) return -1;
        h->mc_active = lag && h->cg_split;
        const int rpw = nc >= 192 ? 4 : 1;
        const int border_lds = (int)((size_t)rpw * D * nc * sizeof(double));
        if (ensure_dynamic_lds((const void*)k_coarse_border<D>, (size_t)border_lds)) return -1;
        if (lag) {
            const int use = h->lci_next;
            h->lci_cur = use;
            const CoarseRhsArgs ra{h->slo, h->shi, h->pnode, h->pw0, h->pw1, h->LciT2[use], h->tvec, h->cg_r[0], h->cg_w[0],
                                   h->cg_s[0], h->cg_p, h->cg_xh, h->cg_split ? 0 : 2, h->lag_status, h->status, h->bgv, h->cg_split ? h->Mc : nullptr};
            hipLaunchKernelGGL(k_coarse_border<D>, dim3(cdiv(nr, rpw) + ncb + 1), dim3(256), border_lds, h->stream,
                               nr, ncb, h->SZ, h->Lci2[use], h->arow_ptr, h->fine_nnz, h->Saug, h->cg_split ? 0 : 1, h->Ac, ra, rpw);
            HIP_OK(hipEventRecord(h->ev_ac, h->stream));
            HIP_OK(hipStreamWaitEvent(h->side, h->ev_ac, 0));
            if (launch_chol(h->side, use ^ 1, h->lag_status)) return -1;
            HIP_OK(hipEventRecord(h->ev_chol, h->side));
            h->lci_next = use ^ 1; h->side_pending = true;
        } else {
            const int buf = h->lci_cur;
            if (launch_chol(h->stream, buf, h->status)) return -1;
            if (h->lagx_ok)
                hipLaunchKernelGGL(k_coarse_xbuild<D>, dim3(cdiv((long)nr * D * nc, 256)), dim3(256), 0, h->stream, nr, ncb,
                                   h->pnode, h->pw0, h->pw1, h->Bmat, h->Lci2[buf], h->X2[buf]);
            const CoarseRhsArgs ra{h->slo, h->shi, h->pnode, h->pw0, h->pw1, h->LciT2[buf], h->tvec, h->cg_r[0], h->cg_w[0],
                                   h->cg_s[0], h->cg_p, h->cg_xh, h->cg_split ? 0 : 1, nullptr, h->status, h->bgv, nullptr};
            hipLaunchKernelGGL(k_coarse_border<D>, dim3(cdiv(nr, rpw) + 1), dim3(256), border_lds, h->stream,
                               nr, ncb, h->SZ, h->Lci2[buf], h->arow_ptr, h->fine_nnz, h->Saug, h->cg_split ? 0 : 1,
                               (const double*)nullptr, ra, rpw);
            h->lci_next = buf;
        }
    }
    h->cg_launched = 0;
    return 0;
}

template <int D>
int cg_side_kick(ps_problem* h) {
    if (!h->side_todo || !h->side_ready) return 0;
    h->side_todo = false;
    const int nr = h->nr, ncb = h->ncb, nc = h->nc, nb = h->side_buf;
    hipLaunchKernelGGL(k_coarse_rowsums<D>, dim3(nr), dim3(256), (size_t)(ncb + 1) * D * D * sizeof(double), h->side,
                       nr, ncb, h->run_lo, h->run_hi, h->acol_idx, h->pnode, h->pw0, h->pw1, h->SB, h->SZ, h->Bmat2[nb], h->BSZ);
    hipLaunchKernelGGL(k_coarse_matrix<D>, dim3(cdiv((long)ncb * ncb * D * D, 256)), dim3(256), 0, h->side,
                       nr, ncb, h->slo, h->shi, h->pnode, h->pw0, h->pw1, h->BSZ, h->Ac);
    if (coarse_factor<D>(h, h->side, nb, h->lag_status)) return -1;
    hipLaunchKernelGGL(k_coarse_xbuild<D>, dim3(cdiv((long)nr * D * nc, 256)), dim3(256), 0, h->side, nr, ncb,
                       h->pnode, h->pw0, h->pw1, h->Bmat2[nb], h->Lci2[nb], h->X2[nb]);
    HIP_OK(hipEventRecord(h->ev_chol, h->side));
    h->lci_next = nb; h->side_pending = true;
    return 0;
}

int side_kick(ps_problem* h) {
    if (!h->side_todo) return 0;
    return h->D == 6 ? cg_side_kick<6>(h) : cg_side_kick<3>(h);
}

template <int D>
void cg_fused_launch(ps_problem* h, double tol, int count) {
    const int cap = h->hist_cap;
    const int rows = h->cg_split ? h->nr : h->nr_aug;
    const int ncbs = h->cg_split ? h->ncb : 0;
    const double tol2 = tol * tol;
#ifdef PS_MEASURE
    if (ps_env("PS_CP_CLOCKS") && !h->cp_dbg) { hipMalloc(&h->cp_dbg, 64); hipMemset(h->cp_dbg, 0, 64); }
#endif
    if (h->cg_persist && h->cp_ok && h->G > 0 && h->cg_lds && !h->cg_split && !h->cg_two_level_reduce &&
        !h->cg_ablate && h->cg_launched == 0 && h->cg_max_launches > 0 && h->cg_max_launches <= 4090 && !h->no_repeat &&
// ... 75 lines not shown
        snprintf(buf, sizeof buf, "CG breakdown: the reduced system is not positive definite (iteration %d, relative residual %.2e)",
                 h->h_status[ST_PCG_ITERS], rr0 > 0.0 ? std::sqrt(rrf / rr0) : 0.0);
        return fail(buf);
    }
    return 0;
}

template <int D>
int cg_fused_run(ps_problem* h, double tol, int max_iters, int* iters_out, double* relres_out, bool rhs_only = false) {
    const int nvec = h->nr * D;
    double* xacc = h->q;
    double* gsaved = h->z;
    int restarts = 0, total_its = 0;
    double reduced = 1.0;
    bool rhs = rhs_only;
    for (;;) {
        const bool forced = h->cg_force_restart && restarts == 0;
        const double tol_pass = forced ? std::max(1e-4, tol) : std::min(0.1, tol / reduced);
        if (cg_fused_setup<D>(h, max_iters, false, rhs)) return -1;
        int chunk = std::max(h->pcg_chunk, h->last_pcg_iters + 2);
        bool done = false;
        while (!done) {
            const int m = std::min(chunk, max_iters + 2 - h->cg_launched);
            cg_fused_launch<D>(h, tol_pass, m);
            HIP_OK(hipMemcpyAsync(h->h_status, h->status, ST_NWORDS * sizeof(int32_t), hipMemcpyDeviceToHost, h->stream));
            HIP_OK(hipMemcpyAsync(h->h_scalars, h->scalars, SC_NWORDS * sizeof(double), hipMemcpyDeviceToHost, h->stream));
            HIP_OK(hipStreamSynchronize(h->stream));
            h->persist_release();
            if (h->h_status[ST_PERSIST_FAIL] && h->cg_persist) { h->cg_persist = 0; ++h->cp_failures; }
            done = h->h_status[ST_PCG_DONE] != 0 || h->cg_launched >= max_iters + 2;
            chunk = h->pcg_chunk;
        }
        total_its += h->h_status[ST_PCG_ITERS];
        const bool pretend = forced && h->h_status[ST_PCG_DONE] == 1 && tol_pass > tol;
        if ((h->h_status[ST_PCG_DONE] != 2 && !pretend) || h->h_status[ST_DIAG_FAIL] || h->h_status[ST_LM_FAIL]) break;
        const double rr0 = h->h_scalars[SC_RR0], rrf = h->h_scalars[SC_RRFINAL];
        const double rho = rr0 > 0.0 ? std::sqrt(rrf / rr0) : 1.0;
        ++h->cg_fallbacks;
        if (restarts == 3 || !(rho < 0.5)) {
            if (restarts) copy_doubles(h->stream, h->g, gsaved, (size_t)nvec);
            return pcg_run<D>(h, tol, max_iters, iters_out, relres_out);
        }
        cg_fused_recover<D>(h, nullptr);
        if (restarts == 0) copy_doubles(h->stream, gsaved, h->g, (size_t)nvec);
        hipLaunchKernelGGL(k_vec_accumulate, dim3(cdiv(nvec, 256)), dim3(256), 0, h->stream, nvec, (const double*)h->x, xacc, restarts == 0);
        hipLaunchKernelGGL(k_bsr_residual<D>, dim3(cdiv(nvec, 256)), dim3(256), 0, h->stream, h->nr, h->row_ptr, h->col_idx, h->S,
                           (const double*)xacc, (const double*)gsaved, h->g);
        reduced *= rho;
        rhs = true;
        ++restarts;
    }
    cg_fused_recover<D>(h, nullptr);
    if (restarts) {
        hipLaunchKernelGGL(k_vec_accumulate, dim3(cdiv(nvec, 256)), dim3(256), 0, h->stream, nvec, (const double*)xacc, h->x, 0);
        copy_doubles(h->stream, h->g, gsaved, (size_t)nvec);
    }
    int its = 0; double rel = 0.0;
    const int rc = cg_report(h, &its, &rel);
    if (iters_out) *iters_out = total_its;
    if (relres_out) *relres_out = rel * reduced;
    h->last_pcg_iters = total_its;
    return rc;
}

int linearize(ps_problem* h, double lambda, bool allow_prelm) {
    h->solver_touched = true;
    h->prelin_valid = false;
    const bool lm_done = allow_prelm && h->prelm_valid && h->prelm_lambda == lambda && h->nv > 0;
    h->prelm_valid = false;
    h->lin_lmfail_tag = lm_done ? h->prelm_tag : 0;
    if (lm_done) ++h->prelm_used;
    h->lin_lambda = lambda;
    h->params_moved_since_lin = false; h->z_foreign = false;
    ++h->prof_tick;
    h->cov_ready = false;
    cov_release(h);
    h->status_clean = false;
    if (h->ldi_sread_pending) {
        HIP_OK(hipStreamWaitEvent(h->stream, h->ev_ldi_sread, 0));
        h->ldi_sread_pending = false;
    }
    const bool zero_by_list = h->lin_zero_gate;
    const bool lm_here = h->nv > 0 && !lm_done;
    if (!zero_by_list) {
        HIP_OK(hipMemsetAsync(h->red, 0, h->red_count * sizeof(double) + ST_NWORDS * sizeof(int32_t), h->stream));
        ++h->lin_fills;
    } else {
        if (lm_here) HIP_OK(hipMemsetAsync(h->status, 0, ST_NWORDS * sizeof(int32_t), h->stream));
        ++h->lin_zero_launches;
    }
    if (lm_here) {
        StageTimer t(h, PS_ST_LANDMARK);
        const ObsWide wl{h->sidx_l, h->stiff_tab};
#define PS_LM_LAUNCH(W) hipLaunchKernelGGL(k_landmark_pass<W>, dim3(cdiv(h->nv, 256 / PS_LM_GROUP)), dim3(256), 0, h->stream, h->nv, h->lm_ptr, \
                           h->lm_point, h->lobs, h->poses, h->points, h->pose_rid, h->ogroups, lambda, h->Z,                       \
                           h->Cinv, h->cvec, h->status, h->lm_ablate, wl)
#define PS_LMP_LAUNCH(W) hipLaunchKernelGGL((k_landmark_pass_packed<W, false>), dim3(cdiv(h->lmw_nwaves, 4)), dim3(256), 0, h->stream, h->lmw_nwaves, \
                           h->lmw_first, h->lm_ptr, h->lm_point, h->lobs, h->poses, h->points, h->pose_rid, h->ogroups, lambda, h->Z,      \
                           h->Cinv, h->cvec, h->status, wl, (const int32_t*)nullptr, (double*)nullptr, (long long*)nullptr, 0LL)
        if (h->lm_packed && h->lmw_nwaves > 0 && !h->lm_ablate) { if (h->wide_obs) PS_LMP_LAUNCH(true); else PS_LMP_LAUNCH(false); }
        else if (h->wide_obs) PS_LM_LAUNCH(true); else PS_LM_LAUNCH(false);
#undef PS_LMP_LAUNCH
#undef PS_LM_LAUNCH
    }
    bool fin_in_combine = false, fin_in_pairs = false;
    static const bool schur_split_env = ps_env("PS_SCHUR_SPLIT") != nullptr;
    if (h->npitems > 0) {
        StageTimer t(h, PS_ST_POSE);
        const ObsWide wp{h->sidx_p, h->stiff_tab};
        const int per_xcd = h->pose_xcd ? cdiv(h->npitems, 8) : 0;
        const int nblk = per_xcd ? 8 * per_xcd : h->npitems;
        static_assert(ST_NWORDS % 2 == 0, "the status words are cleared as doubles");
        const int ntail = zero_by_list ? h->nr * 6 + 2 + (lm_here ? 0 : ST_NWORDS / 2) : 0;
        const int nzs = zero_by_list ? h->nzero_slots : 0;
        const int nzblk = zero_by_list ? cdiv((long)nzs * 36 + ntail, 256) : 0;
        if (h->wide_obs)
            hipLaunchKernelGGL(k_pose_pass<true>, dim3(nblk + nzblk), dim3(256), 0, h->stream, h->pitems, h->pobs,
                               h->poses, h->points, h->ogroups, h->Cinv, h->cvec, h->ppartial, lambda != 0.0 ? 1 : 0, wp, h->npitems, per_xcd,
                               nblk, (const int32_t*)h->zero_slots, nzs, h->S, h->g, ntail);
        else
            hipLaunchKernelGGL(k_pose_pass<false>, dim3(nblk + nzblk), dim3(256), 0, h->stream, h->pitems, h->pobs,
                               h->poses, h->points, h->ogroups, h->Cinv, h->cvec, h->ppartial, lambda != 0.0 ? 1 : 0, wp, h->npitems, per_xcd,
                               nblk, (const int32_t*)h->zero_slots, nzs, h->S, h->g, ntail);
        fin_in_combine = h->Spart && h->npair_items > 0 && !h->has_diag_tasks && h->D == 6;
        fin_in_pairs = !h->Spart && h->schur_pipeline && h->npair_items > 0 && !h->has_diag_tasks && h->D == 6 && !schur_split_env;
        if (!fin_in_combine && !fin_in_pairs)
            hipLaunchKernelGGL(k_pose_finalize, dim3(h->nr), dim3(64), 0, h->stream, h->nr, h->pitem_ptr,
                               h->ppartial, h->diag_slot, lambda, h->S, h->g);
    }
    if (h->npair_items > 0) {
        StageTimer t(h, PS_ST_SCHUR, 1);
        const bool split2 = schur_split_env;
        const int halfp = split2 ? (h->pair_per_xcd / 2 + 3) / 4 * 4 : h->pair_per_xcd;
        static const int lds_pad = ps_env("PS_SCHUR_LDS_PAD") ? atoi(ps_env("PS_SCHUR_LDS_PAD")) : 0;
        auto launch_pairs = [&](int nblk, int lds, int from, int to) {
            if (!h->schur_pipeline)
                hipLaunchKernelGGL(k_schur_pairs, dim3(nblk), dim3(256), lds, h->stream, h->pair_per_xcd, h->pair_xitems, h->pairs,
                                   h->Z, h->S, h->Spart, h->schur_ablate, from, to);
            else {
#ifdef PS_MEASURE
                auto k = h->schur_ablate == 0 ? k_schur_pairs_db<0> : h->schur_ablate == 1 ? k_schur_pairs_db<1> :
                         h->schur_ablate == 2 ? k_schur_pairs_db<2> : h->schur_ablate == 3 ? k_schur_pairs_db<3> :
                         h->schur_ablate == 4 ? k_schur_pairs_db<4> : k_schur_pairs_db<5>;
#else
                auto k = k_schur_pairs_db<0>;
#endif
                hipLaunchKernelGGL(k, dim3(nblk + (fin_in_pairs ? cdiv(h->nr, 4) : 0)), dim3(256), lds, h->stream, h->pair_per_xcd,
                                   h->pair_xitems, h->pairs, h->Z, h->S, h->Spart, from, to, nblk, fin_in_pairs ? h->nr : 0,
                                   h->pitem_ptr, h->ppartial, h->diag_slot, lambda, h->g);
            }
        };
        launch_pairs(8 * (halfp / 4), lds_pad, 0, halfp);
        if (split2 && halfp < h->pair_per_xcd) launch_pairs(8 * ((h->pair_per_xcd - halfp + 3) / 4), 0, halfp, h->pair_per_xcd);
        if (h->Spart)
            hipLaunchKernelGGL(k_schur_combine, dim3(cdiv(h->ncomb, 4) + (fin_in_combine ? cdiv(h->nr, 4) : 0)), dim3(256), 0,
                               h->stream, h->ncomb, h->comb_items, h->comb_tasks, h->Spart, h->S,
                               fin_in_combine ? h->nr : 0, h->pitem_ptr, h->ppartial, h->diag_slot, lambda, h->g);
    }
    if ((h->F > 0 || h->FH > 0) && h->nr > 0) {
        StageTimer t(h, PS_ST_EDGES);
        if (h->D == 6) launch_factor_pass<6>(h, lambda); else launch_factor_pass<3>(h, lambda);
    }
    return side_kick(h);
}

inline bool cost_packed_possible(const ps_problem* h) {
    return h->fuse_cost != 0 && h->lm_packed && h->lmw_nwaves > 0 && !h->lm_ablate && h->Nl == h->N && h->nv > 0 && h->D == 6;
}
int cost_partials_pass(ps_problem* h, int include_all, const int32_t* gate) {
    int n = 0;
    if (h->N > 0 && include_all && cost_packed_possible(h)) {
        const ObsWide wl{h->sidx_l, h->stiff_tab};
        const int nbl = cdiv(h->lmw_nwaves, 4);
        if (h->wide_obs)
            hipLaunchKernelGGL(k_cost_packed<true>, dim3(nbl), dim3(256), 0, h->stream, h->lmw_nwaves, h->lmw_first, h->lm_ptr, h->lm_point,
                               h->lobs, h->poses, h->points, h->ogroups, h->cost_partials, gate, wl);
        else
            hipLaunchKernelGGL(k_cost_packed<false>, dim3(nbl), dim3(256), 0, h->stream, h->lmw_nwaves, h->lmw_first, h->lm_ptr, h->lm_point,
                               h->lobs, h->poses, h->points, h->ogroups, h->cost_partials, gate, wl);
        n += nbl;
    } else if (h->N > 0) {
        const ObsWide wl{h->sidx_l, h->stiff_tab};
        if (h->wide_obs)
            hipLaunchKernelGGL(k_cost_reproj<true>, dim3(h->ncost_obs), dim3(256), 0, h->stream, h->N, h->lobs, h->poses,
                               h->points, h->pose_rid, h->point_vid, h->ogroups, include_all, h->cost_partials, gate, wl);
        else
            hipLaunchKernelGGL(k_cost_reproj<false>, dim3(h->ncost_obs), dim3(256), 0, h->stream, h->N, h->lobs, h->poses,
                               h->points, h->pose_rid, h->point_vid, h->ogroups, include_all, h->cost_partials, gate, wl);
        n += h->ncost_obs;
    }
    if (h->F > 0) {
        if (h->D == 6)
            hipLaunchKernelGGL(k_cost_factors<6>, dim3(h->ncost_fac), dim3(256), 0, h->stream, (int)h->F, h->f_i,
                               h->f_j, h->f_Tinv, h->f_grp, h->fgroups, h->poses, h->pose_rid, include_all,
                               h->cost_partials + n, gate);
        else
            hipLaunchKernelGGL(k_cost_factors<3>, dim3(h->ncost_fac), dim3(256), 0, h->stream, (int)h->F, h->f_i,
                               h->f_j, h->f_Tinv, h->f_grp, h->fgroups, h->poses, h->pose_rid, include_all,
                               h->cost_partials + n, gate);
        n += h->ncost_fac;
    }
    return n;
}

int cost_pass(ps_problem* h, int include_all, int scalar_slot) {
    StageTimer t(h, PS_ST_COST);
    const int n = cost_partials_pass(h, include_all, nullptr);
    hipLaunchKernelGGL(k_reduce_partials, dim3(1), dim3(256), 0, h->stream, n, h->cost_partials,
                       h->scalars + scalar_slot);
    return 0;
}

inline int nsq_l_now(const ps_problem* h) { return (h->lm_packed && h->lmw_nwaves > 0) ? cdiv(h->lmw_nwaves, 4) : h->nsq_l16; }

int lm_md_ensure(ps_problem* h) {
    if (h->md_part_p) return 0;
    h->nmd_p = std::max(1, cdiv((long)h->nr * h->D + (long)h->nes * h->D, 256));
    return (h->alloc(&h->md_part_p, (size_t)h->nmd_p) || h->alloc(&h->md_part_l, (size_t)std::max({h->nsq_l, h->nsq_l16, 1}))) ? -1 : 0;
}

int backsub(ps_problem* h, const int32_t* gate = nullptr, bool fuse_update = false, long long* hearly = nullptr, long long eseq = 0) {
    if (h->nv == 0) return 0;
    StageTimer t(h, PS_ST_BACKSUB);
    const double lam_ratio = h->lin_lambda / (1.0 + h->lin_lambda);
    if (h->lm_packed && h->lmw_nwaves > 0) {
        const int nbl = cdiv(h->lmw_nwaves, 4);
#define PS_BSP_LAUNCH(MD, ...) hipLaunchKernelGGL(k_backsub_packed<MD>, dim3(nbl + (fuse_update ? h->nsq_p : 0)), dim3(256), 0, h->stream, h->lmw_nwaves, \
                               h->lmw_first, h->lm_ptr, h->Z, h->Cinv, h->cvec, h->x, h->dxl, h->sq_part_l, gate, nbl, __VA_ARGS__)
        if (h->lm_md) {
            if (fuse_update) PS_BSP_LAUNCH(true, h->lm_point, h->points, h->P, h->pose_rid, h->poses, h->sq_part_p, hearly, eseq, h->md_part_l, lam_ratio);
            else PS_BSP_LAUNCH(true, (const int32_t*)nullptr, (double*)nullptr, 0, (const int32_t*)nullptr, (double*)nullptr, (double*)nullptr, hearly, eseq,
                               h->md_part_l, lam_ratio);
        } else if (fuse_update)
            PS_BSP_LAUNCH(false, h->lm_point, h->points, h->P, h->pose_rid, h->poses, h->sq_part_p, hearly, eseq);
        else
            PS_BSP_LAUNCH(false, (const int32_t*)nullptr, (double*)nullptr, 0, (const int32_t*)nullptr, (double*)nullptr, (double*)nullptr, hearly, eseq);
#undef PS_BSP_LAUNCH
        return 0;
    }
#define PS_BS_LAUNCH(MD, ...) hipLaunchKernelGGL(k_backsub<MD>, dim3(h->nsq_l16 + (fuse_update ? h->nsq_p : 0)), dim3(256), 0, h->stream, h->nv, h->lm_ptr, \
                               h->lobs, h->pose_rid, h->Z, h->Cinv, h->cvec, h->x, h->dxl, h->sq_part_l, gate, h->nsq_l16, __VA_ARGS__)
    if (h->lm_md) {
        if (fuse_update) PS_BS_LAUNCH(true, h->lm_point, h->points, h->P, h->poses, h->sq_part_p, hearly, eseq, h->md_part_l, lam_ratio);
        else PS_BS_LAUNCH(true, (const int32_t*)nullptr, (double*)nullptr, 0, (double*)nullptr, (double*)nullptr, hearly, eseq, h->md_part_l, lam_ratio);
    } else if (fuse_update)
        PS_BS_LAUNCH(false, h->lm_point, h->points, h->P, h->poses, h->sq_part_p, hearly, eseq);
    else
        PS_BS_LAUNCH(false, (const int32_t*)nullptr, (double*)nullptr, 0, (double*)nullptr, (double*)nullptr, hearly, eseq);
#undef PS_BS_LAUNCH
    return 0;
}

int lm_md_enqueue(ps_problem* h, const int32_t* gate) {
    const int32_t* pip = h->npitems > 0 ? h->pitem_ptr : nullptr;
#define PS_LMP_SUMS(DD) hipLaunchKernelGGL(k_lm_pose_sums<DD>, dim3(h->nmd_p), dim3(256), 0, h->stream, h->nr, h->x, h->g, pip, h->ppartial, h->nes,   \
                               h->eslots, h->eptr, h->eitems, h->eslot_diag, h->brow_of, h->fscratch, h->lin_lambda, gate, h->md_part_p)
    if (h->D == 6) PS_LMP_SUMS(6); else PS_LMP_SUMS(3);
#undef PS_LMP_SUMS
    hipLaunchKernelGGL(k_lm_total, dim3(1), dim3(256), 0, h->stream, h->nmd_p, h->md_part_p, h->nv > 0 ? nsq_l_now(h) : 0, h->md_part_l, gate,
                       h->scalars + SC_MODELDEC);
    return 0;
}

int step_norm(ps_problem* h) {
    double* part = h->cost_partials;
    HIP_OK(hipMemsetAsync(h->scalars + SC_DXP2, 0, sizeof(double), h->stream));
    HIP_OK(hipMemsetAsync(h->scalars + SC_DXL2, 0, sizeof(double), h->stream));
    if (h->nr > 0) {
        const int b = std::min(256, cdiv((long)h->nr * h->D, 256));
        hipLaunchKernelGGL(k_sumsq_partials, dim3(b), dim3(256), 0, h->stream, (long)h->nr * h->D, h->x, 1.0, part);
        hipLaunchKernelGGL(k_reduce_partials, dim3(1), dim3(256), 0, h->stream, b, part, h->scalars + SC_DXP2);
    }
    if (h->nv > 0) {
        const int b = std::min(256, cdiv((long)h->nv * 3, 256));
        hipLaunchKernelGGL(k_sumsq_partials, dim3(b), dim3(256), 0, h->stream, (long)h->nv * 3, h->dxl, 1.0, part + 256);
        hipLaunchKernelGGL(k_reduce_partials, dim3(1), dim3(256), 0, h->stream, b, part + 256, h->scalars + SC_DXL2);
    }
    return 0;
}

int apply_update(ps_problem* h, double step, const int32_t* gate = nullptr, bool with_norm = false, long long* hearly = nullptr, long long eseq = 0) {
    h->params_moved_since_lin = true;
    h->prelin_valid = h->prelm_valid = false;
    StageTimer t(h, PS_ST_UPDATE);
    if (h->nr > 0) {
        double* sq = with_norm ? h->sq_part_p : nullptr;
        if (h->D == 6)
            hipLaunchKernelGGL(k_update_poses<6>, dim3(cdiv(h->P, 256)), dim3(256), 0, h->stream, h->P, h->pose_rid, h->x, step, h->poses, sq, gate, hearly, eseq);
        else
            hipLaunchKernelGGL(k_update_poses<3>, dim3(cdiv(h->P, 256)), dim3(256), 0, h->stream, h->P, h->pose_rid, h->x, step, h->poses, sq, gate, hearly, eseq);
    }
    if (h->nv > 0)
        hipLaunchKernelGGL(k_update_points, dim3(cdiv((long)h->nv * 3, 256)), dim3(256), 0, h->stream, h->nv,
                           h->lm_point, h->dxl, step, h->points, gate);
    return 0;
}

inline bool lm_cost_possible(const ps_problem* h) {
    return cost_packed_possible(h) && (!h->shard_out || (h->nccl_allreduce && h->nccl_comm));
}
int lm_cost_enqueue(ps_problem* h, double lambda, const int32_t* gate) {
    const int nbl = cdiv(h->lmw_nwaves, 4);
    if (h->params_moved_since_lin || lambda != h->lin_lambda) h->z_foreign = true;
    h->prelm_tag = ++h->prelm_seq;
    {
        StageTimer t(h, PS_ST_LANDMARK);
        const ObsWide wl{h->sidx_l, h->stiff_tab};
#define PS_LMC_LAUNCH(W) hipLaunchKernelGGL((k_landmark_pass_packed<W, true>), dim3(nbl), dim3(256), 0, h->stream, h->lmw_nwaves, h->lmw_first,    \
                           h->lm_ptr, h->lm_point, h->lobs, h->poses, h->points, h->pose_rid, h->ogroups, lambda, h->Z, h->Cinv, h->cvec,        \
                           h->status, wl, gate, h->cost_partials, h->h_lmfail_dev + (h->prelm_tag & 1), h->prelm_tag)
        if (h->wide_obs) PS_LMC_LAUNCH(true); else PS_LMC_LAUNCH(false);
#undef PS_LMC_LAUNCH
    }
    int n = nbl;
    if (h->F > 0) {
        StageTimer t(h, PS_ST_COST);
        hipLaunchKernelGGL(k_cost_factors<6>, dim3(h->ncost_fac), dim3(256), 0, h->stream, (int)h->F, h->f_i, h->f_j, h->f_Tinv, h->f_grp,
                           h->fgroups, h->poses, h->pose_rid, 1, h->cost_partials + nbl, gate);
        n += h->ncost_fac;
    }
    h->prelm_lambda = lambda;
    return n;
}
int lm_cost_pass(ps_problem* h, double lambda, int scalar_slot) {
    h->prelin_valid = false;
    const int n = lm_cost_enqueue(h, lambda, nullptr);
    hipLaunchKernelGGL(k_reduce_partials, dim3(1), dim3(256), 0, h->stream, n, h->cost_partials, h->scalars + scalar_slot);
    h->prelm_pending = false; h->prelm_valid = true;
    return 0;
}

int gn_tail(ps_problem* h, int linesearch, const int32_t* gate, bool publish = false) {
    h->params_moved_since_lin = true;
    h->prelin_valid = h->prelm_valid = false;
    h->prelm_pending = false;
    const bool fused = linesearch && h->nv > 0 && h->nr > 0 && h->D == 6;
    long long* const hearly = (publish && h->spec_next && !h->spec_enqueued && gate) ? h->h_early_dev : nullptr;
    const long long eseq = hearly ? ++h->early_seq : 0;
    h->early_armed = hearly != nullptr;
    const bool stamp_in_backsub = h->nv > 0;
    if (h->lm_md && lm_md_ensure(h)) return -1;
    if (backsub(h, gate, fused, stamp_in_backsub ? hearly : nullptr, eseq)) return -1;
    if (h->lm_md && lm_md_enqueue(h, gate)) return -1;
    int ncost = 0;
    if (!linesearch) { StageTimer t(h, PS_ST_COST); ncost = cost_partials_pass(h, 0, gate); }
    if (!fused && apply_update(h, 1.0, gate, true, stamp_in_backsub ? nullptr : hearly, eseq)) return -1;
    if (!stamp_in_backsub && (fused || h->nr == 0)) h->early_armed = false;
    const bool lm_cost = fused && (publish || (h->shard_out && h->nccl_allreduce && h->nccl_comm)) && h->expect_next && lm_cost_possible(h);
    if (lm_cost) {
        ncost = lm_cost_enqueue(h, h->lin_lambda, gate);
        h->prelm_pending = true;
    } else if (linesearch) { StageTimer t(h, PS_ST_COST); ncost = cost_partials_pass(h, 1, gate); }
    double* o_cost = h->shard_out ? h->shard_buf : h->scalars + (linesearch ? SC_COST : SC_LINCOST);
    double* o_dxl = h->shard_out ? h->shard_buf + 1 : h->scalars + SC_DXL2;
    hipLaunchKernelGGL(k_reduce3, dim3(3), dim3(256), 0, h->stream,
                       ncost, h->cost_partials, o_cost,
                       h->nsq_p, h->sq_part_p, h->nr > 0 ? h->scalars + SC_DXP2 : nullptr,
                       nsq_l_now(h), h->sq_part_l, (h->nv > 0 || h->shard_out) ? o_dxl : nullptr, gate,
                       h->status, h->scalars, publish ? h->h_status_dev : nullptr, publish ? h->h_scalars_dev : nullptr,
                       h->arrivals, publish ? h->h_seq_dev : nullptr, publish ? ++h->seq : 0LL);
    return 0;
}

}
```

pyslam_amd/csrc/ps_k_cg_fused.h:

```cpp
#pragma once

template <int D>
__global__ __launch_bounds__(256) void k_block_jacobi_factor(
    int nr, const int32_t* __restrict__ diag_slot, const double* __restrict__ S,
    double* __restrict__ Linv, int32_t* __restrict__ status,
    const double* __restrict__ g, double* __restrict__ r0, double* __restrict__ w0, double* __restrict__ s0,
    double* __restrict__ p0, double* __restrict__ x0,
    const double* __restrict__ poses, const int32_t* __restrict__ pose_of_rid, int basis,
    double* __restrict__ Bmat, double* __restrict__ bg)
{
    constexpr int DD = D * D;
    __shared__ double sA[4][DD], sLi[4][DD], sB[4][DD], sR[4][D];
    const int wv = threadIdx.x >> 6, lane = threadIdx.x & 63;
    const int i = blockIdx.x * 4 + wv;
    if (g && blockIdx.x == 0 && threadIdx.x == 0) { status[ST_PCG_DONE] = 0; status[ST_PCG_ITERS] = 0; }
    if (i >= nr) return;
    const bool act = lane < DD;
    const int r = act ? lane / D : 0, c = act ? lane % D : 0;
    double* A = sA[wv];
    double* Li = sLi[wv];
    if (act) { A[lane] = S[(size_t)diag_slot[i] * DD + lane]; Li[lane] = 0.0; }
    __builtin_amdgcn_wave_barrier();
    bool ok = true;
#pragma unroll
    for (int j = 0; j < D; ++j) {
        const double d = A[j * D + j];
        ok = ok && (d > 0.0);
        const double l = sqrt(d);
        __builtin_amdgcn_wave_barrier();
        if (act && c == j && r >= j) A[lane] = (r == j) ? l : A[lane] / l;
        __builtin_amdgcn_wave_barrier();
        if (act && r > j && c > j) A[lane] -= A[r * D + j] * A[c * D + j];
        __builtin_amdgcn_wave_barrier();
    }
    if (lane < D) {
        const int cc = lane;
        double col[D];
#pragma unroll
        for (int rr = 0; rr < D; ++rr) {
            double v = (rr == cc) ? 1.0 : 0.0;
#pragma unroll
            for (int k = 0; k < rr; ++k) v -= (k >= cc) ? A[rr * D + k] * col[k] : 0.0;
            col[rr] = (rr >= cc) ? v / A[rr * D + rr] : 0.0;
            Li[rr * D + cc] = col[rr];
        }
    }
    __builtin_amdgcn_wave_barrier();
    if (!ok && lane == 0) atomicAdd(&status[ST_DIAG_FAIL], 1);
    if (act) Linv[(size_t)i * DD + lane] = Li[lane];
    if (g && lane < D) {
        double v = 0.0;
#pragma unroll
        for (int k = 0; k < D; ++k) v += Li[lane * D + k] * g[(size_t)i * D + k];
        const size_t o = (size_t)i * D + lane;
        r0[o] = v; w0[o] = 0.0; s0[o] = 0.0; p0[o] = 0.0; x0[o] = 0.0;
        sR[wv][lane] = v;
    }
    if (!Bmat) return;
    if (act) {
        typedef PoseOps<D> G;
        double v = (r == c) ? 1.0 : 0.0;
        if (basis == 1) {
            const double* Tp = poses + G::W * (size_t)pose_of_rid[i];
            v = 0.0;
#pragma unroll
            for (int m2 = 0; m2 < D; ++m2) v += (m2 >= r) ? A[m2 * D + r] * G::adj_mem(Tp, m2, c) : 0.0;
        }
        Bmat[(size_t)i * DD + lane] = v;
        sB[wv][lane] = v;
    }
    __builtin_amdgcn_wave_barrier();
    if (g && lane < D) {
        double v = 0.0;
#pragma unroll
        for (int a = 0; a < D; ++a) v += sB[wv][a * D + lane] * sR[wv][a];
        bg[(size_t)i * D + lane] = v;
    }
}

template <int D>
__global__ __launch_bounds__(64) void k_scale_blocks(
    int nr, const int32_t* __restrict__ row_ptr, const int32_t* __restrict__ col_idx,
    const int32_t* __restrict__ brow_of, const double* __restrict__ Linv, const double* __restrict__ S,
    const int32_t* __restrict__ out_slot, double* __restrict__ Sout,
    const double* __restrict__ Bmat ,
    double* __restrict__ SB)
{
    constexpr int DD = D * D;
    __shared__ double sS[36], sT[36], sLi[36], sLj[36], sB[36];
    const int b = blockIdx.x, t = threadIdx.x;
    const int i = brow_of[b], j = col_idx[b];
    if (t < DD) {
        sS[t] = S[(size_t)b * DD + t];
        sLi[t] = Linv[(size_t)i * DD + t];
        sLj[t] = Linv[(size_t)j * DD + t];
        if (Bmat) sB[t] = Bmat[(size_t)j * DD + t];
    }
    __syncthreads();
    const int r = t / D, c = t % D;
    if (t < DD) {
        double v = 0.0;
#pragma unroll
        for (int a = 0; a < D; ++a) v += sLi[r * D + a] * sS[a * D + c];
        sT[t] = v;
    }
    __syncthreads();
    if (t < DD) {
        double v = 0.0;
#pragma unroll
        for (int a = 0; a < D; ++a) v += sT[r * D + a] * sLj[c * D + a];
        Sout[(size_t)out_slot[b] * DD + t] = v;
        sS[t] = v;
    }
    if (!Bmat) return;
    __syncthreads();
    if (t < DD) {
        double v = 0.0;
#pragma unroll
        for (int a = 0; a < D; ++a) v += sS[r * D + a] * sB[a * D + c];
        SB[(size_t)out_slot[b] * DD + t] = v;
    }
}

#define PS_SCB_NB 4
template <int D>
__global__ __launch_bounds__(256) void k_scale_blocks_p(
    int nnzb, const int32_t* __restrict__ col_idx, const int32_t* __restrict__ brow_of,
    const double* __restrict__ Linv, const double* __restrict__ S, const int32_t* __restrict__ out_slot,
    double* __restrict__ Sout, const double* __restrict__ Bmat, double* __restrict__ SB)
{
    constexpr int DD = D * D;
    __shared__ double lds[4][5][36];
    const int wv = threadIdx.x >> 6, t = threadIdx.x & 63;
    const int b0 = (blockIdx.x * 4 + wv) * PS_SCB_NB;
    if (b0 >= nnzb) return;
    double *sS = lds[wv][0], *sT = lds[wv][1], *sLi = lds[wv][2], *sLj = lds[wv][3], *sB = lds[wv][4];
    int bi[PS_SCB_NB], bj[PS_SCB_NB], bs[PS_SCB_NB];
#pragma unroll
    for (int q = 0; q < PS_SCB_NB; ++q) {
        const int b = min(b0 + q, nnzb - 1);
        bi[q] = brow_of[b]; bj[q] = col_idx[b]; bs[q] = out_slot[b];
    }
    double vs[PS_SCB_NB], vi[PS_SCB_NB], vj[PS_SCB_NB], vb[PS_SCB_NB];
    const int tt = t < DD ? t : 0;
#pragma unroll
    for (int q = 0; q < PS_SCB_NB; ++q) {
        const int b = min(b0 + q, nnzb - 1);
        vs[q] = S[(size_t)b * DD + tt];
        vi[q] = Linv[(size_t)bi[q] * DD + tt];
        vj[q] = Linv[(size_t)bj[q] * DD + tt];
        vb[q] = Bmat ? Bmat[(size_t)bj[q] * DD + tt] : 0.0;
    }
    const int r = tt / D, c = tt % D;
#pragma unroll
    for (int q = 0; q < PS_SCB_NB; ++q) {
        if (b0 + q >= nnzb) break;
        if (t < DD) { sS[t] = vs[q]; sLi[t] = vi[q]; sLj[t] = vj[q]; sB[t] = vb[q]; }
        __builtin_amdgcn_wave_barrier();
        double v = 0.0;
#pragma unroll
// ... 643 lines not shown
```

pyslam_amd/csrc/ps_k_linearize.h:

```cpp
#pragma once

#define PS_LM_GROUP 16

PS_DEV double group16_sum(double v) {
    v = dpp_shift_add<0x111, 0xf, 0xf>(v);
    v = dpp_shift_add<0x112, 0xf, 0xf>(v);
    v = dpp_shift_add<0x114, 0xf, 0xe>(v);
    v = dpp_shift_add<0x118, 0xf, 0xc>(v);
    return __shfl(v, (int)(threadIdx.x & 63) | 15, 64);
}

#define PS_ZROW 16

PS_DEV void lm_emit_m(const ReprojEval& ev, double M00, double M10, double M11, double M20, double M21,
                      double M22, double* __restrict__ m) {
#pragma unroll
    for (int a = 0; a < 3; ++a) {
        const double w0 = ev.Jp[a] * ev.Jl[0] + ev.Jp[6 + a] * ev.Jl[3] + ev.Jp[12 + a] * ev.Jl[6];
        const double w1 = ev.Jp[a] * ev.Jl[1] + ev.Jp[6 + a] * ev.Jl[4] + ev.Jp[12 + a] * ev.Jl[7];
        const double w2 = ev.Jp[a] * ev.Jl[2] + ev.Jp[6 + a] * ev.Jl[5] + ev.Jp[12 + a] * ev.Jl[8];
        m[3 * a] = w0 * M00;
        m[3 * a + 1] = w0 * M10 + w1 * M11;
        m[3 * a + 2] = w0 * M20 + w1 * M21 + w2 * M22;
    }
// ... 196 lines not shown
    for (int i = it.start + threadIdx.x; i < it.end; i += 256) {
        const LObs o = pobs[i];
        const int v = PS_POSE_OF(o) - 1;
        const double pw[3] = {points[3 * (size_t)o.point], points[3 * (size_t)o.point + 1], points[3 * (size_t)o.point + 2]};
        double m[6] = {0, 0, 0, 0, 0, 0}, c0 = 0.0, c1 = 0.0, c2 = 0.0;
        if (v >= 0) {
            const double* ci = Cinv + 6 * (size_t)v;
#pragma unroll
            for (int k = 0; k < 6; ++k) m[k] = ci[k];
            c0 = cvec[3 * (size_t)v]; c1 = cvec[3 * (size_t)v + 1]; c2 = cvec[3 * (size_t)v + 2];
        }
        ReprojEval ev;
        reproj_eval_obs<true, true, WIDE>(T, pw, &o.u, groups, PS_GRP_OF(o), wide, i, ev);
        double G[6], t3[3];
        {
            const double* J = ev.Jp;
            G[0] = J[0] * J[0] + J[6] * J[6] + J[12] * J[12];
            G[1] = J[0] * J[1] + J[6] * J[7] + J[12] * J[13];
            G[2] = J[0] * J[2] + J[6] * J[8] + J[12] * J[14];
            G[3] = J[1] * J[1] + J[7] * J[7] + J[13] * J[13];
            G[4] = J[1] * J[2] + J[7] * J[8] + J[13] * J[14];
            G[5] = J[2] * J[2] + J[8] * J[8] + J[14] * J[14];
#pragma unroll
            for (int a = 0; a < 3; ++a) t3[a] = J[a] * ev.r[0] + J[6 + a] * ev.r[1] + J[12 + a] * ev.r[2];
        }
        if (want_diag) {
            double d21[21];
#pragma unroll
            for (int k = 0; k < 21; ++k) d21[k] = 0.0;
            pose_sandwich(G, ev.pc, d21);
            acc[27] += d21[0]; acc[28] += d21[6]; acc[29] += d21[11]; acc[30] += d21[15]; acc[31] += d21[18]; acc[32] += d21[20];
        }
        if (v >= 0) {
            double m9[9];
            lm_emit_m(ev, m[0], m[1], m[2], m[3], m[4], m[5], m9);
            G[0] -= m9[0] * m9[0] + m9[1] * m9[1] + m9[2] * m9[2];
            G[1] -= m9[0] * m9[3] + m9[1] * m9[4] + m9[2] * m9[5];
            G[2] -= m9[0] * m9[6] + m9[1] * m9[7] + m9[2] * m9[8];
            G[3] -= m9[3] * m9[3] + m9[4] * m9[4] + m9[5] * m9[5];
            G[4] -= m9[3] * m9[6] + m9[4] * m9[7] + m9[5] * m9[8];
            G[5] -= m9[6] * m9[6] + m9[7] * m9[7] + m9[8] * m9[8];
#pragma unroll
            for (int a = 0; a < 3; ++a) t3[a] += m9[3 * a] * c0 + m9[3 * a + 1] * c1 + m9[3 * a + 2] * c2;
        }
        pose_sandwich(G, ev.pc, acc);
        acc[21] -= t3[0]; acc[22] -= t3[1]; acc[23] -= t3[2];
        acc[24] -= ev.pc[1] * t3[2] - ev.pc[2] * t3[1];
        acc[25] -= ev.pc[2] * t3[0] - ev.pc[0] * t3[2];
        acc[26] -= ev.pc[0] * t3[1] - ev.pc[1] * t3[0];
    }
#if PS_POSE_TRANSPOSE
    {
        double* trw = tr[w];
#pragma unroll
        for (int h2 = 0; h2 < 2; ++h2) {
            const int k0 = 17 * h2, nk = h2 ? PS_NPOSE_ACC - 17 : 17;
#pragma unroll
            for (int k = 0; k < 17; ++k) if (k < nk) trw[lane * 17 + k] = acc[k0 + k];
            __builtin_amdgcn_wave_barrier();
            if (lane < nk) {
                double s = 0.0;
#pragma unroll 8
                for (int l = 0; l < 64; ++l) s += trw[l * 17 + lane];
                red[w][k0 + lane] = s;
            }
            __builtin_amdgcn_wave_barrier();
        }
    }
#else
#pragma unroll
    for (int k = 0; k < PS_NPOSE_ACC; ++k) {
        const double s = wave_sum(acc[k]);
        if (lane == 0) red[w][k] = s;
    }
#endif
    __syncthreads();
    if (threadIdx.x < PS_NPOSE_ACC)
        partial[(size_t)item * PS_NPOSE_ACC + threadIdx.x] =
            ((red[0][threadIdx.x] + red[1][threadIdx.x]) + red[2][threadIdx.x]) + red[3][threadIdx.x];
}

PS_DEV void pose_finalize_wave(int rid, int lane, const int32_t* __restrict__ pitem_ptr,
                               const double* __restrict__ partial, const int32_t* __restrict__ diag_slot,
                               double lambda, double* __restrict__ S, double* __restrict__ g, double* v )
{
    if (lane < PS_NPOSE_ACC) {
        double s = 0.0;
        for (int it = pitem_ptr[rid]; it < pitem_ptr[rid + 1]; ++it) s += partial[(size_t)it * PS_NPOSE_ACC + lane];
        v[lane] = s;
    }
    __builtin_amdgcn_wave_barrier();
    if (lane < 36) {
        const int r = lane / 6, c = lane % 6;
        const int a = r < c ? r : c, b = r < c ? c : r;
        const int idx = a * 6 - (a * (a - 1)) / 2 + (b - a);
        double val = v[idx];
        if (r == c) val += lambda * v[27 + r];
        S[(size_t)diag_slot[rid] * 36 + lane] += val;
    }
    if (lane < 6) g[(size_t)rid * 6 + lane] += v[21 + lane];
}

__global__ __launch_bounds__(64) void k_pose_finalize(
    int nr, const int32_t* __restrict__ pitem_ptr, const double* __restrict__ partial,
    const int32_t* __restrict__ diag_slot, double lambda,
    double* __restrict__ S, double* __restrict__ g)
{
    __shared__ double v[PS_NPOSE_ACC];
    pose_finalize_wave(blockIdx.x, threadIdx.x, pitem_ptr, partial, diag_slot, lambda, S, g, v);
}

#ifndef PS_SP_WAVES
#define PS_SP_WAVES 4
#endif
#define PS_SP_PAIRS 32
#define PS_SP_ROWD 14
#define PS_SP_LDS_PER_WAVE (64 * PS_SP_ROWD)

PS_DEV double half_sum_dpp(double v) {
    v = dpp_shift_add<0x111, 0xf, 0xf>(v);
    v = dpp_shift_add<0x112, 0xf, 0xf>(v);
    v = dpp_shift_add<0x114, 0xf, 0xe>(v);
    v = dpp_shift_add<0x118, 0xf, 0xc>(v);
    v = dpp_shift_add<0x142, 0xa, 0xf>(v);
    return v;
}

__global__ __launch_bounds__(256) __attribute__((amdgpu_waves_per_eu(PS_SP_WAVES, 8))) void k_schur_pairs(
    int per_xcd, const PairItem* __restrict__ xitems ,
    const int2* __restrict__ pairs, const double* __restrict__ Z, double* __restrict__ S,
    double* __restrict__ Spart , int ablate,
    int first , int last)
{
    __shared__ __attribute__((aligned(16))) double smem[4 * PS_SP_LDS_PER_WAVE];
    const int lane = threadIdx.x & 63, wv = threadIdx.x >> 6;
    double* rows = smem + wv * PS_SP_LDS_PER_WAVE;
    const int local = first + (blockIdx.x >> 3) * 4 + wv;
    if (local >= last) return;
    const size_t pos = (size_t)(blockIdx.x & 7) * per_xcd + local;
    const PairItem it = xitems[pos];
    if (it.slot < 0) return;
    const int p = lane & 31, hf = lane >> 5;
    const int slot = lane / 7, piece = lane - 7 * slot;
    const int32_t* flat = reinterpret_cast<const int32_t*>(pairs) + hf;
    double acc[18];
#pragma unroll
    for (int k = 0; k < 18; ++k) acc[k] = 0.0;
    int mine = (it.start + p < it.end) ? flat[2 * (size_t)(it.start + p)] : -1;
    int mine1 = (it.start + PS_SP_PAIRS + p < it.end) ? flat[2 * (size_t)(it.start + PS_SP_PAIRS + p)] : -1;
    for (int base = it.start; base < it.end; base += PS_SP_PAIRS) {
        const int n = min(PS_SP_PAIRS, it.end - base);
        int zrow[8];
#pragma unroll
        for (int k = 0; k < 8; ++k) zrow[k] = __shfl(mine, (9 * k + slot) & 63, 64);
        const int nb = base + 2 * PS_SP_PAIRS;
        const int mine2 = (nb + p < it.end) ? flat[2 * (size_t)(nb + p)] : -1;
#pragma unroll
        for (int k = 0; k < 8; ++k) {
            const int r = 9 * k + slot;
            if (slot < 9 && r < 2 * PS_SP_PAIRS && zrow[k] >= 0 && !(ablate & 2) && !((ablate & 4) && r < PS_SP_PAIRS))
                __builtin_amdgcn_global_load_lds((ps_gptr_t)(Z + PS_ZROW * (size_t)zrow[k] + 2 * piece),
                                                 (ps_lptr_t)(rows + 9 * PS_SP_ROWD * k), 16, 0, 0);
        }
        __builtin_amdgcn_s_waitcnt(0x0F70);
        __builtin_amdgcn_wave_barrier();
        if (p < n && !(ablate & 1)) {
            double A[9];
            {
                double ma[12];
                const double2* pa = reinterpret_cast<const double2*>(rows + PS_SP_ROWD * p);
#pragma unroll
                for (int k = 0; k < 6; ++k) { const double2 va = pa[k]; ma[2 * k] = va.x; ma[2 * k + 1] = va.y; }
                zrow_cross(ma, ma + 9, A);
#pragma unroll
                for (int k = 0; k < 9; ++k) A[k] = hf ? A[k] : ma[k];
            }
            double mb[12];
            const double2* pb = reinterpret_cast<const double2*>(rows + PS_SP_ROWD * (PS_SP_PAIRS + p));
#pragma unroll
            for (int k = 0; k < 6; ++k) { const double2 vb = pb[k]; mb[2 * k] = vb.x; mb[2 * k + 1] = vb.y; }
#pragma unroll
            for (int a = 0; a < 3; ++a)
#pragma unroll
// ... 187 lines not shown
```

pyslam_amd/csrc/ps_k_schur2.h:

```cpp
#pragma once

#define PS_SQ_ROWD 12
#define PS_SQ_BUF (64 * PS_SQ_ROWD)
#define PS_SQ_BUFSTEP (4 * PS_SQ_BUF * 8)

typedef double ps_d2 __attribute__((ext_vector_type(2)));
#ifndef PS_SQ_ASM_CLOBBER
#define PS_SQ_ASM_CLOBBER "memory"
#endif

PS_DEV void sq_fetch_idx(const int32_t* __restrict__ src , int32_t* slot ) {
    __builtin_amdgcn_global_load_lds((ps_gptr_t)src, (ps_lptr_t)slot, 4, 0, 0);
}

template <bool HOT >
PS_DEV void sq_fetch(const double* __restrict__ Z, const uint32_t (&ia)[6], uint32_t slot_off, double* buf, const int (&off_of)[6]) {
    int zr[6];
    asm volatile(
        "ds_read_b32 %0, %6\n\t"
        "ds_read_b32 %1, %7\n\t"
        "ds_read_b32 %2, %8\n\t"
        "ds_read_b32 %3, %9\n\t"
        "ds_read_b32 %4, %10\n\t"
        "ds_read_b32 %5, %11\n\t"
        "s_waitcnt lgkmcnt(0)"
        : "=&v"(zr[0]), "=&v"(zr[1]), "=&v"(zr[2]), "=&v"(zr[3]), "=&v"(zr[4]), "=&v"(zr[5])
        : "v"(ia[0] + slot_off), "v"(ia[1] + slot_off), "v"(ia[2] + slot_off), "v"(ia[3] + slot_off), "v"(ia[4] + slot_off),
          "v"(ia[5] + slot_off)
        : "memory");
#pragma unroll
    for (int k = 0; k < 6; ++k) {
        if (HOT) zr[k] &= 63;
        __builtin_amdgcn_global_load_lds((ps_gptr_t)(Z + PS_ZROW * (size_t)zr[k] + off_of[k]), (ps_lptr_t)(buf + 128 * k), 16, 0, 0);
    }
}

PS_DEV void sq_products(uint32_t aa, uint32_t ab, int hf, double (&acc)[18]) {
    ps_d2 va[6], vb[6];
    asm volatile(
        "ds_read_b128 %0, %12\n\t"
        "ds_read_b128 %1, %12 offset:16\n\t"
        "ds_read_b128 %2, %12 offset:32\n\t"
        "ds_read_b128 %3, %12 offset:48\n\t"
        "ds_read_b128 %4, %12 offset:64\n\t"
        "ds_read_b128 %5, %12 offset:80\n\t"
        "ds_read_b128 %6, %13\n\t"
        "ds_read_b128 %7, %13 offset:16\n\t"
        "ds_read_b128 %8, %13 offset:32\n\t"
        "ds_read_b128 %9, %13 offset:48\n\t"
        "ds_read_b128 %10, %13 offset:64\n\t"
        "ds_read_b128 %11, %13 offset:80\n\t"
        "s_waitcnt lgkmcnt(0)"
        : "=&v"(va[0]), "=&v"(va[1]), "=&v"(va[2]), "=&v"(va[3]), "=&v"(va[4]), "=&v"(va[5]),
          "=&v"(vb[0]), "=&v"(vb[1]), "=&v"(vb[2]), "=&v"(vb[3]), "=&v"(vb[4]), "=&v"(vb[5])
        : "v"(aa), "v"(ab)
        : PS_SQ_ASM_CLOBBER);
    double A[9];
    {
        double ma[12];
#pragma unroll
        for (int k = 0; k < 6; ++k) { ma[2 * k] = va[k].x; ma[2 * k + 1] = va[k].y; }
        zrow_cross(ma, ma + 9, A);
#pragma unroll
        for (int k = 0; k < 9; ++k) A[k] = hf ? A[k] : ma[k];
    }
    double mb[12];
#pragma unroll
    for (int k = 0; k < 6; ++k) { mb[2 * k] = vb[k].x; mb[2 * k + 1] = vb[k].y; }
#pragma unroll
    for (int a = 0; a < 3; ++a)
#pragma unroll
        for (int b = 0; b < 3; ++b)
            acc[6 * a + b] += A[3 * a] * mb[3 * b] + A[3 * a + 1] * mb[3 * b + 1] + A[3 * a + 2] * mb[3 * b + 2];
    double Lb[9];
    zrow_cross(mb, mb + 9, Lb);
#pragma unroll
    for (int a = 0; a < 3; ++a)
#pragma unroll
        for (int b = 0; b < 3; ++b)
            acc[6 * a + 3 + b] += A[3 * a] * Lb[3 * b] + A[3 * a + 1] * Lb[3 * b + 1] + A[3 * a + 2] * Lb[3 * b + 2];
}

#define PS_SQ_WAIT_CHUNK() __builtin_amdgcn_s_waitcnt(0x0F70 | 7)
#define PS_SQ_WAIT_ALL() __builtin_amdgcn_s_waitcnt(0x0F70)

template <int ABL >
__global__ __launch_bounds__(256) __attribute__((amdgpu_waves_per_eu(3, 3))) void k_schur_pairs_db(
    int per_xcd, const PairItem* __restrict__ xitems, const int2* __restrict__ pairs, const double* __restrict__ Z,
    double* __restrict__ S, double* __restrict__ Spart, int first, int last,
    int fin_first_block, int fin_nr, const int32_t* __restrict__ pitem_ptr, const double* __restrict__ ppartial,
    const int32_t* __restrict__ diag_slot, double lambda, double* __restrict__ g)
{
    constexpr int ablate = ABL;
    __shared__ __attribute__((aligned(16))) double sbuf[2 * 4 * PS_SQ_BUF];
    __shared__ __attribute__((aligned(16))) int32_t sidx[4 * 256];
    const int lane = threadIdx.x & 63, wv = threadIdx.x >> 6;
    double* const buf0 = sbuf + wv * PS_SQ_BUF;
    double* const buf1 = buf0 + 4 * PS_SQ_BUF;
    int32_t* const islot = sidx + wv * 256;
    if ((int)blockIdx.x >= fin_first_block) {
        const int rid = ((int)blockIdx.x - fin_first_block) * 4 + wv;
        if (rid < fin_nr) pose_finalize_wave(rid, lane, pitem_ptr, ppartial, diag_slot, lambda, S, g, buf0);
        return;
    }
    const int local = first + (blockIdx.x >> 3) * 4 + wv;
    if (local >= last) return;
    const size_t pos = (size_t)(blockIdx.x & 7) * per_xcd + local;
    PairItem it = xitems[pos];
    it.slot = __builtin_amdgcn_readfirstlane(it.slot); it.slotT = __builtin_amdgcn_readfirstlane(it.slotT);
    it.start = __builtin_amdgcn_readfirstlane(it.start); it.end = __builtin_amdgcn_readfirstlane(it.end);
    if (it.slot < 0) return;
    const int p = lane & 31, hf = lane >> 5;
    const int32_t* flat = reinterpret_cast<const int32_t*>(pairs) + hf;
    uint32_t ia[6];
    int off_of[6];
#pragma unroll
    for (int k = 0; k < 6; ++k) {
        const int q = 64 * k + lane, row = q / 6;
        ia[k] = (uint32_t)(uintptr_t)(ps_lptr_t)(islot + row);
        off_of[k] = 2 * (q - 6 * row);
    }
    const uint32_t aa = (uint32_t)(uintptr_t)(ps_lptr_t)(buf0 + PS_SQ_ROWD * p), ab = aa + 32 * PS_SQ_ROWD * 8;
    double acc[18];
#pragma unroll
    for (int k = 0; k < 18; ++k) acc[k] = 0.0;
    const int npairs = it.end - it.start, nch = (npairs + 31) >> 5, last_pair = max(it.end - 1, 0);
#define PS_SQ_IDX(c) (flat + 2 * (size_t)min(it.start + 32 * (c) + p, last_pair))
    sq_fetch_idx(PS_SQ_IDX(0), islot + 0);
    sq_fetch_idx(PS_SQ_IDX(1), islot + 64);
    sq_fetch_idx(PS_SQ_IDX(2), islot + 128);
    PS_SQ_WAIT_ALL();
    __builtin_amdgcn_wave_barrier();
    if (!(ablate & 2)) sq_fetch<(ABL & 4) != 0>(Z, ia, 0, buf0, off_of);
    sq_fetch_idx(PS_SQ_IDX(3), islot + 192);
    if (nch > 1 && !(ablate & 2)) sq_fetch<(ABL & 4) != 0>(Z, ia, 256, buf1, off_of);
    int c = 0;
    for (; c + 2 < nch; ++c) {
        const uint32_t boff = (c & 1) * PS_SQ_BUFSTEP;
        PS_SQ_WAIT_CHUNK();
        __builtin_amdgcn_wave_barrier();
        if (!(ablate & 1)) sq_products(aa + boff, ab + boff, hf, acc);
        __builtin_amdgcn_wave_barrier();
        sq_fetch_idx(PS_SQ_IDX(c + 4), islot + 64 * (c & 3));
        if (!(ablate & 2)) sq_fetch<(ABL & 4) != 0>(Z, ia, 256 * ((c + 2) & 3), (c & 1) ? buf1 : buf0, off_of);
    }
    if (c + 1 < nch) {
        PS_SQ_WAIT_CHUNK();
        __builtin_amdgcn_wave_barrier();
        if (!(ablate & 1)) sq_products(aa + (c & 1) * PS_SQ_BUFSTEP, ab + (c & 1) * PS_SQ_BUFSTEP, hf, acc);
        __builtin_amdgcn_wave_barrier();
        ++c;
    }
    {
        PS_SQ_WAIT_ALL();
        __builtin_amdgcn_wave_barrier();
        if (p < npairs - 32 * c && !(ablate & 1)) sq_products(aa + (c & 1) * PS_SQ_BUFSTEP, ab + (c & 1) * PS_SQ_BUFSTEP, hf, acc);
        __builtin_amdgcn_wave_barrier();
    }
#undef PS_SQ_IDX
    double* sums = buf0;
#pragma unroll
    for (int k = 0; k < 18; ++k) {
        const double t = half_sum_dpp(acc[k]);
        if (p == 31) sums[18 * hf + k] = t;
    }
    __builtin_amdgcn_wave_barrier();
    if (lane < 36) {
        const int r = lane / 6, cc = lane % 6;
        const double mine_v = sums[lane];
        if (Spart) {
            Spart[pos * 36 + lane] = mine_v;
        } else if (it.slot == it.slotT) {
            S[(size_t)it.slot * 36 + lane] -= mine_v + sums[cc * 6 + r];
        } else {
            S[(size_t)it.slot * 36 + lane] = -mine_v;
            S[(size_t)it.slotT * 36 + cc * 6 + r] = -mine_v;
        }
    }
}
```

pyslam_amd/csrc/ps_kernels.h:

```cpp
#pragma once
#include "ps_math.h"
#include "ps_limits.h"

struct __attribute__((aligned(32))) LObs {
    double u, v, d;
    int32_t pose_grp;
    int32_t point;
};
struct PItem { int32_t rid, start, end, pad; };
struct PairItem { int32_t slot, slotT, start, end; };
struct FactorGroup { double S[36]; int32_t loss_id; int32_t pad; double loss_k; };

#define PS_POSE_OF(o) ((o).pose_grp & 0xFFFFFF)
#define PS_GRP_OF(o) (((uint32_t)(o).pose_grp) >> 24)

enum { ST_LM_FAIL = 0, ST_DIAG_FAIL = 1, ST_PCG_DONE = 2, ST_PCG_ITERS = 3, ST_PERSIST_FAIL = 4 , ST_NWORDS = 8 };
enum { SC_COST = 0, SC_DXP2 = 1, SC_LINCOST = 2, SC_RR0 = 3, SC_RRFINAL = 4, SC_THRESH = 5, SC_DXL2 = 6, SC_STARTCOST = 7, SC_MODELDEC = 8, SC_NWORDS = 9 };

template <int CTRL, int ROW_MASK, int BANK_MASK>
PS_DEV double dpp_shift_add(double v) {
    const unsigned long long b = __builtin_bit_cast(unsigned long long, v);
    const int lo = __builtin_amdgcn_update_dpp(0, (int)(unsigned)b, CTRL, ROW_MASK, BANK_MASK, false);
    const int hi = __builtin_amdgcn_update_dpp(0, (int)(unsigned)(b >> 32), CTRL, ROW_MASK, BANK_MASK, false);
    const unsigned long long m = ((unsigned long long)(unsigned)hi << 32) | (unsigned)lo;
    return v + __builtin_bit_cast(double, m);
}

PS_DEV double wave_sum(double v) {
    v = dpp_shift_add<0x111, 0xf, 0xf>(v);
    v = dpp_shift_add<0x112, 0xf, 0xf>(v);
    v = dpp_shift_add<0x114, 0xf, 0xe>(v);
    v = dpp_shift_add<0x118, 0xf, 0xc>(v);
    v = dpp_shift_add<0x142, 0xa, 0xf>(v);
    v = dpp_shift_add<0x143, 0xc, 0xf>(v);
    const unsigned long long b = __builtin_bit_cast(unsigned long long, v);
    const unsigned lo = __builtin_amdgcn_readlane((int)(unsigned)b, 63);
    const unsigned hi = __builtin_amdgcn_readlane((int)(unsigned)(b >> 32), 63);
    return __builtin_bit_cast(double, ((unsigned long long)hi << 32) | lo);
}

PS_DEV double block_sum(double v, double* lds ) {
    v = wave_sum(v);
    const int w = threadIdx.x >> 6, nw = blockDim.x >> 6;
    __syncthreads();
    if ((threadIdx.x & 63) == 0) lds[w] = v;
    __syncthreads();
    double t = 0.0;
    for (int i = 0; i < nw; ++i) t += lds[i];
    return t;
}

PS_DEV void block_sum2(double& a, double& b, double* lds ) {
    a = wave_sum(a); b = wave_sum(b);
    const int w = threadIdx.x >> 6, nw = blockDim.x >> 6;
    __syncthreads();
    if ((threadIdx.x & 63) == 0) { lds[w] = a; lds[16 + w] = b; }
    __syncthreads();
    double sa = 0.0, sb = 0.0;
    for (int i = 0; i < nw; ++i) { sa += lds[i]; sb += lds[16 + i]; }
    a = sa; b = sb;
}

#include "ps_k_linearize.h"
#include "ps_k_schur2.h"
#include "ps_k_pcg_classic.h"
#include "ps_k_ldi.h"
#include "ps_k_cg_fused.h"
#include "ps_k_cg_persist.h"
#include "ps_k_xcg.h"
#include "ps_k_xcg_persist.h"
#include "ps_k_coarse.h"
#include "ps_k_band.h"
#include "ps_k_bandpart.h"
#include "ps_k_lm.h"
#include "ps_k_tail.h"
#include "ps_k_packed.h"
```

Measured before the change: 0.2917.

## Fuse block-Jacobi preconditioner factorization into Schur pair kernel's pose-finalize waves

Moves the per-pose 6x6 block-Jacobi Cholesky/inverse (plus basis and RHS setup) into the pose-finalize waves of the Schur pairs kernel, placed as leading blocks so they run while pair blocks still execute. The later CG setup then skips its separate k_block_jacobi_factor launch when the recorded plan (lag, basis buffer) matches. This is meant to remove one kernel launch and a reread of the diagonal blocks from memory per LM iteration. In exchange it adds validity tracking that every parameter-changing path must invalidate, and a gate that falls back to the separate launch on mismatch.

Result: faster. 0.2865 (median of 6 runs) (-1.8%).

```diff
diff --git a/pyslam_amd/csrc/ps_abi_problem.h b/pyslam_amd/csrc/ps_abi_problem.h
--- a/pyslam_amd/csrc/ps_abi_problem.h
+++ b/pyslam_amd/csrc/ps_abi_problem.h
@@ -875,7 +875,7 @@
         HIP_OK(hipStreamSynchronize(h->stream));
     }
     h->host_cost = cost;
-    h->prelin_valid = false;
+    h->prelin_valid = h->ride_valid = false;
     h->last_cost = h->prev_cost = -1.0;
     return 0;
 }
diff --git a/pyslam_amd/csrc/ps_abi_solver.h b/pyslam_amd/csrc/ps_abi_solver.h
--- a/pyslam_amd/csrc/ps_abi_solver.h
+++ b/pyslam_amd/csrc/ps_abi_solver.h
@@ -74,7 +74,7 @@
 
 int ps_shard_unpack(ps_problem* h) {
     if (!h) return fail("null argument");
-    h->prelin_valid = h->prelm_valid = false;
+    h->prelin_valid = h->prelm_valid = h->ride_valid = false;
     if (ensure_shard_pack(h)) return -1;
     const long ntail = (long)h->nr * h->D + 2;
     const int nb = (int)std::min<long>(4096, cdiv(h->pack_count, 256));
@@ -133,7 +133,7 @@
 
 int ps_apply_update(ps_problem* h, double step) {
     if (!h) return fail("null argument");
-    h->prelin_valid = h->prelm_valid = false;
+    h->prelin_valid = h->prelm_valid = h->ride_valid = false;
     h->last_cost = h->prev_cost = -1.0;
     return apply_update(h, step);
 }
@@ -152,7 +152,7 @@
 static int restore_params_by_exchange(ps_problem* h) {
     if (!h->snap_valid) return fail("ps_solve: no snapshot to restore");
     h->params_moved_since_lin = true;
-    h->prelin_valid = h->prelm_valid = false;
+    h->prelin_valid = h->prelm_valid = h->ride_valid = false;
     h->last_cost = h->snap_cost; h->prev_cost = -1.0;
     std::swap(h->poses, h->poses_snap);
     std::swap(h->points, h->points_snap);
@@ -164,7 +164,7 @@
     if (!h) return fail("null argument");
     if (!h->snap_valid) return fail("ps_restore_params: no snapshot (none taken, or ps_solve has consumed it)");
     h->params_moved_since_lin = true;
-    h->prelin_valid = h->prelm_valid = false;
+    h->prelin_valid = h->prelm_valid = h->ride_valid = false;
     h->last_cost = h->snap_cost; h->prev_cost = -1.0;
     const size_t n1 = (size_t)h->P * h->PW, n2 = (size_t)h->L * 3;
     if (n1 + n2)
@@ -183,7 +183,7 @@
 int ps_set_params(ps_problem* h, const double* poses, const double* points) {
     if (!h) return fail("null argument");
     h->params_moved_since_lin = true;
-    h->prelin_valid = h->prelm_valid = false;
+    h->prelin_valid = h->prelm_valid = h->ride_valid = false;
     h->last_cost = h->prev_cost = -1.0;
     if (poses && h->P) HIP_OK(hipMemcpyAsync(h->poses, poses, (size_t)h->P * h->PW * sizeof(double), hipMemcpyDefault, h->stream));
     if (points && h->L) HIP_OK(hipMemcpyAsync(h->points, points, (size_t)h->L * 3 * sizeof(double), hipMemcpyDefault, h->stream));
@@ -271,7 +271,7 @@
         { StageTimer tpk(h, PS_ST_PACK); if (ps_shard_unpack(h)) return -1; }
         return 0;
     }
-    h->prelin_valid = h->prelm_valid = false;
+    h->prelin_valid = h->prelm_valid = h->ride_valid = false;
     const long T = 3, ntail = (long)h->nr * h->D + 2;
     const unsigned nb1 = (unsigned)std::min<long>(2048, cdiv(h->seg_maxlen, 256)), nb2 = (unsigned)std::min<long>(4096, cdiv(h->seg_ndst + T, 256));
     {
@@ -633,7 +633,7 @@
 int ps_motion_only_solve(ps_problem* h, const ps_solve_options* o, double* cost_history, int32_t cap, int32_t* n_history,
                          int32_t* iterations, double* last_dx_norm, double* pose12_out) {
     if (!h || !o || !cost_history || !n_history) return fail("null argument");
-    h->prelin_valid = h->prelm_valid = false;
+    h->prelin_valid = h->prelm_valid = h->ride_valid = false;
     const bool eligible = h->mo_fused && !h->hybrid && h->nv == 0 && h->F == 0 && h->nr == 1 && h->P == 1 && h->D == 6 && h->N == h->Np &&
                           h->pcg_variant == 1 && h->max_pose_obs <= 2048;
     const int need = o->max_iters + 2;
@@ -676,7 +676,7 @@
     if (!h) return fail("null argument");
     cov_release(h);
     ++h->cov_epoch;
-    h->prelin_valid = h->prelm_valid = false;
+    h->prelin_valid = h->prelm_valid = h->ride_valid = false;
     if (linearize(h, 0.0)) return -1;
     if (h->nr > 0 && h->pcg_variant == 1 && !use_direct(h) && !h->coarse_built && build_coarse(h)) return -1;
     if (h->nr > 0 && h->pcg_variant == 1 && !use_direct(h) && !h->cg_explicit) {
@@ -834,7 +834,13 @@
     if (!h || !name) return fail("null argument");
     if (!std::strcmp(name, "expect_next")) { h->expect_next = value != 0 && !h->hybrid; return 0; }
     if (!std::strcmp(name, "solve_horizon")) { h->solve_horizon = value < 0 ? -1 : (int)std::min(value, 1e6); return 0; }
-    h->prelin_valid = h->prelm_valid = false;
+    if (!std::strcmp(name, "setup_ride")) {
+        h->setup_ride = value != 0 ? 1 : 0;
+        h->prelin_valid = h->prelm_valid = false;
+        relook_launch_gates(h);
+        return 0;
+    }
+    h->prelin_valid = h->prelm_valid = h->ride_valid = false;
     const char* refusal = nullptr;
     const int fx = ps_option_apply(*h, name, value, &refusal);
     if (fx == PS_OPT_UNKNOWN) return fail(std::string("unknown option: ") + name);
@@ -854,13 +860,17 @@
     if (n == "lin_zero_list") *value = h->lin_zero_gate ? 1.0 : 0.0;
     else if (n == "lin_fills") *value = (double)h->lin_fills;
     else if (n == "lin_zero_launches") *value = (double)h->lin_zero_launches;
+    else if (n == "setup_ride") *value = h->ride_gate ? 1.0 : 0.0;
+    else if (n == "factor_launches") *value = (double)h->bjf_launches;
+    else if (n == "factors_ridden") *value = (double)h->bjf_ridden;
+    else if (n == "factor_plan_mismatches") *value = (double)h->bjf_mismatches;
     else return fail("ps_get_option: no read-back for option: " + n);
     return 0;
 }
 
 int ps_reset_solver_state(ps_problem* h) {
     if (!h) return fail("null argument");
-    h->prelin_valid = h->prelm_valid = false;
+    h->prelin_valid = h->prelm_valid = h->ride_valid = false;
     if (!h->solver_touched) {
         static_cast<PsCostHistory&>(*h) = PsCostHistory{};
         return 0;
diff --git a/pyslam_amd/csrc/ps_abi_triang.h b/pyslam_amd/csrc/ps_abi_triang.h
--- a/pyslam_amd/csrc/ps_abi_triang.h
+++ b/pyslam_amd/csrc/ps_abi_triang.h
@@ -47,7 +47,7 @@
                            h->lobs, h->poses, h->points, h->ogroups, wl, refine_iters, cos_min, write_back ? 1 : 0, d_pts, d_status);
     if (write_back) {
         h->params_moved_since_lin = true;
-        h->prelin_valid = h->prelm_valid = false;
+        h->prelin_valid = h->prelm_valid = h->ride_valid = false;
         h->last_cost = h->prev_cost = -1.0;
     }
     std::vector<double> pts(points_out && !vids ? (size_t)n * 3 : 0);
diff --git a/pyslam_amd/csrc/ps_core.hip b/pyslam_amd/csrc/ps_core.hip
--- a/pyslam_amd/csrc/ps_core.hip
+++ b/pyslam_amd/csrc/ps_core.hip
@@ -226,6 +226,11 @@
     bool has_extra_pairs = false;
     bool lin_zero_gate = false;
     long lin_fills = 0, lin_zero_launches = 0;
+    int setup_ride = 1;
+    bool ride_gate = false, ride_valid = false, ride_lagged = false;
+    int ride_use = 0;
+    double* ride_basis = nullptr;
+    long bjf_launches = 0, bjf_ridden = 0, bjf_mismatches = 0;
     std::vector<int32_t> h_row_ptr, h_col_idx;
     std::vector<int32_t> h_vid_of_slot;
     double *x = nullptr, *r = nullptr, *z = nullptr, *p0 = nullptr, *p1 = nullptr, *q = nullptr, *Minv = nullptr;
@@ -519,6 +524,10 @@
 inline void relook_launch_gates(ps_problem* h) {
     const bool shard = (h->nccl_allreduce && h->nccl_comm) || h->seg_allgather || h->shard_pack || h->has_extra_pairs;
     h->lin_zero_gate = h->lin_zero_list && h->zero_slots && !h->Spart && h->schur_pipeline && h->npitems > 0 && h->D == 6 && !shard;
+    h->ride_gate = h->setup_ride && !h->Spart && h->schur_pipeline && h->npitems > 0 && h->npair_items > 0 && !h->has_diag_tasks &&
+                   h->D == 6 && h->F == 0 && h->FH == 0 && !shard && h->pcg_variant == 1 && h->nr > 0 &&
+                   h->nr * h->D > h->direct_max && !(h->coarse_built && h->cg_explicit);
+    h->ride_valid = false;
 }
 
 #include "ps_host_cg.h"
diff --git a/pyslam_amd/csrc/ps_host_cg.h b/pyslam_amd/csrc/ps_host_cg.h
--- a/pyslam_amd/csrc/ps_host_cg.h
+++ b/pyslam_amd/csrc/ps_host_cg.h
@@ -42,6 +42,7 @@
 int side_kick(ps_problem* h);
 int ldi_side_kick(ps_problem* h);
 int linearize(ps_problem* h, double lambda, bool allow_prelm = false);
+bool use_direct(const ps_problem* h);
 
 void drain_timers_ready(ps_problem* h) {
     std::vector<std::pair<int, int>> keep;
@@ -591,11 +592,28 @@
     return 0;
 }
 
+struct CgSetupPlan { bool lagged; int use; double* basis_out; };
+inline CgSetupPlan cg_setup_plan(const ps_problem* h, bool allow_lag, int lci_next) {
+    CgSetupPlan p{};
+    p.lagged = h->G && h->lagx_ok && h->lagx && allow_lag && h->coarse_lag && lci_next >= 0;
+    if (p.lagged) { p.use = lci_next; p.basis_out = h->Bmat2[lci_next ^ 1]; }
+    else { p.use = h->lagx_ok ? h->lci_cur : 0; p.basis_out = h->G ? h->Bmat2[p.use] : nullptr; }
+    return p;
+}
+
+inline bool ride_consume(ps_problem* h, const CgSetupPlan& plan) {
+    if (!h->ride_valid) return false;
+    h->ride_valid = false;
+    if (plan.lagged == h->ride_lagged && plan.use == h->ride_use && plan.basis_out == h->ride_basis) return true;
+    ++h->bjf_mismatches;
+    return false;
+}
+
 template <int D>
 int cg_fused_setup(ps_problem* h, int max_iters, bool allow_lag = false, bool rhs_only = false) {
     const int nr = h->nr, cap = h->hist_cap;
     if (max_iters + 2 > cap) return fail("pcg max_iters exceeds the history buffer (4096)");
-    if (!h->coarse_built && build_coarse(h)) return -1;
+    if (!h->coarse_built) { h->ride_valid = false; if (build_coarse(h)) return -1; }
     h->cg_max_launches = max_iters + 2;
     h->cp_recovered = false;
     h->cg_two_level_reduce = h->nr_aug > 2048 || h->cg_split;
@@ -619,14 +637,18 @@
         HIP_OK(hipStreamWaitEvent(h->stream, h->ev_chol, 0));
         h->side_pending = false;
     }
-    if (G && h->lagx_ok && h->lagx && allow_lag && h->coarse_lag && h->lci_next >= 0) {
+    const CgSetupPlan plan = cg_setup_plan(h, allow_lag, h->lci_next);
+    const bool ridden = ride_consume(h, plan);
+    if (!ridden) ++h->bjf_launches;
+    if (plan.lagged) {
         const int ncb = h->ncb, nc = h->nc;
-        const int use = h->lci_next, nb = use ^ 1;
+        const int use = plan.use, nb = use ^ 1;
         h->lci_cur = use;
         h->Bmat = h->Bmat2[use];
-        hipLaunchKernelGGL(k_block_jacobi_factor<D>, dim3(cdiv(nr, 4)), dim3(256), 0, h->stream, nr, h->diag_slot,
-                           h->S, h->Linv, h->status, h->g, h->cg_r[0], h->cg_w[0], h->cg_s[0], h->cg_p, h->cg_xh,
-                           h->poses, h->pose_of_rid, h->coarse_basis, h->Bmat2[nb], h->bgv);
+        if (!ridden)
+            hipLaunchKernelGGL(k_block_jacobi_factor<D>, dim3(cdiv(nr, 4)), dim3(256), 0, h->stream, nr, h->diag_slot,
+                               h->S, h->Linv, h->status, h->g, h->cg_r[0], h->cg_w[0], h->cg_s[0], h->cg_p, h->cg_xh,
+                               h->poses, h->pose_of_rid, h->coarse_basis, plan.basis_out, h->bgv);
         if (!h->rows_attr_set) {
             if (ensure_dynamic_lds((const void*)k_rows_setup<D>, (size_t)(h->rows_lds))) return -1;
             h->rows_attr_set = true;
@@ -647,10 +669,11 @@
     }
     h->last_setup_lagx = false;
     h->side_todo = false;
-    if (G) h->Bmat = h->Bmat2[h->lagx_ok ? h->lci_cur : 0];
-    hipLaunchKernelGGL(k_block_jacobi_factor<D>, dim3(cdiv(nr, 4)), dim3(256), 0, h->stream, nr, h->diag_slot,
-                       h->S, h->Linv, h->status, h->g, h->cg_r[0], h->cg_w[0], h->cg_s[0], h->cg_p, h->cg_xh,
-                       h->poses, h->pose_of_rid, h->coarse_basis, G ? h->Bmat : (double*)nullptr, h->bgv);
+    if (G) h->Bmat = plan.basis_out;
+    if (!ridden)
+        hipLaunchKernelGGL(k_block_jacobi_factor<D>, dim3(cdiv(nr, 4)), dim3(256), 0, h->stream, nr, h->diag_slot,
+                           h->S, h->Linv, h->status, h->g, h->cg_r[0], h->cg_w[0], h->cg_s[0], h->cg_p, h->cg_xh,
+                           h->poses, h->pose_of_rid, h->coarse_basis, plan.basis_out, h->bgv);
     hipLaunchKernelGGL(k_scale_blocks<D>, dim3(h->nnzb), dim3(64), 0, h->stream, nr, h->row_ptr, h->col_idx,
                        h->brow_of, h->Linv, h->S, h->aug_slot, h->Saug, G ? h->Bmat : (const double*)nullptr, h->SB);
     if (G) {
@@ -892,6 +915,24 @@
     }
     const bool zero_by_list = h->lin_zero_gate;
     const bool lm_here = h->nv > 0 && !lm_done;
+    BjFactorOut ride{};
+    h->ride_valid = false;
+    if (h->ride_gate && h->nr > 0 && h->pcg_variant == 1 && !use_direct(h)) {
+        if (!h->coarse_built && build_coarse(h)) return -1;
+        if (h->cg_explicit) h->ride_gate = false;
+        else {
+            const int lci = (h->side_todo && h->side_ready) ? h->side_buf : h->lci_next;
+            const CgSetupPlan plan = cg_setup_plan(h, allow_prelm, lci);
+            const CgSetupPlan lag = cg_setup_plan(h, true, lci);
+            const bool held = plan.basis_out && ((lag.lagged && plan.basis_out == h->Bmat2[lag.use]) ||
+                                                 (h->side_todo && plan.basis_out == h->Bmat2[h->side_buf]));
+            if (!held) {
+                ride = BjFactorOut{h->Linv, h->status, h->cg_r[0], h->cg_w[0], h->cg_s[0], h->cg_p, h->cg_xh, h->poses, h->pose_of_rid,
+                                   h->coarse_basis, plan.basis_out, h->bgv};
+                h->ride_lagged = plan.lagged; h->ride_use = plan.use; h->ride_basis = plan.basis_out;
+            }
+        }
+    }
     if (!zero_by_list) {
         HIP_OK(hipMemsetAsync(h->red, 0, h->red_count * sizeof(double) + ST_NWORDS * sizeof(int32_t), h->stream));
         ++h->lin_fills;
@@ -955,9 +996,12 @@
 #else
                 auto k = k_schur_pairs_db<0>;
 #endif
-                hipLaunchKernelGGL(k, dim3(nblk + (fin_in_pairs ? cdiv(h->nr, 4) : 0)), dim3(256), lds, h->stream, h->pair_per_xcd,
+                const int nfin = fin_in_pairs ? cdiv(h->nr, 4) : 0;
+                const int lead = (fin_in_pairs && ride.Linv) ? (nfin + 7) / 8 * 8 : 0;
+                hipLaunchKernelGGL(k, dim3(nblk + (lead ? lead : nfin)), dim3(256), lds, h->stream, h->pair_per_xcd,
                                    h->pair_xitems, h->pairs, h->Z, h->S, h->Spart, from, to, nblk, fin_in_pairs ? h->nr : 0,
-                                   h->pitem_ptr, h->ppartial, h->diag_slot, lambda, h->g);
+                                   h->pitem_ptr, h->ppartial, h->diag_slot, lambda, h->g, fin_in_pairs ? ride : BjFactorOut{}, lead);
+                if (fin_in_pairs && ride.Linv) { h->ride_valid = true; ++h->bjf_ridden; }
             }
         };
         launch_pairs(8 * (halfp / 4), lds_pad, 0, halfp);
@@ -1091,7 +1135,7 @@
 
 int apply_update(ps_problem* h, double step, const int32_t* gate = nullptr, bool with_norm = false, long long* hearly = nullptr, long long eseq = 0) {
     h->params_moved_since_lin = true;
-    h->prelin_valid = h->prelm_valid = false;
+    h->prelin_valid = h->prelm_valid = h->ride_valid = false;
     StageTimer t(h, PS_ST_UPDATE);
     if (h->nr > 0) {
         double* sq = with_norm ? h->sq_part_p : nullptr;
@@ -1133,7 +1177,7 @@
     return n;
 }
 int lm_cost_pass(ps_problem* h, double lambda, int scalar_slot) {
-    h->prelin_valid = false;
+    h->prelin_valid = h->ride_valid = false;
     const int n = lm_cost_enqueue(h, lambda, nullptr);
     hipLaunchKernelGGL(k_reduce_partials, dim3(1), dim3(256), 0, h->stream, n, h->cost_partials, h->scalars + scalar_slot);
     h->prelm_pending = false; h->prelm_valid = true;
@@ -1142,7 +1186,7 @@
 
 int gn_tail(ps_problem* h, int linesearch, const int32_t* gate, bool publish = false) {
     h->params_moved_since_lin = true;
-    h->prelin_valid = h->prelm_valid = false;
+    h->prelin_valid = h->prelm_valid = h->ride_valid = false;
     h->prelm_pending = false;
     const bool fused = linesearch && h->nv > 0 && h->nr > 0 && h->D == 6;
     long long* const hearly = (publish && h->spec_next && !h->spec_enqueued && gate) ? h->h_early_dev : nullptr;
diff --git a/pyslam_amd/csrc/ps_k_bjfactor.h b/pyslam_amd/csrc/ps_k_bjfactor.h
--- /dev/null
+++ b/pyslam_amd/csrc/ps_k_bjfactor.h
@@ -0,0 +1,86 @@
+#pragma once
+
+struct BjFactorOut {
+    double* Linv;
+    int32_t* status;
+    double *r0, *w0, *s0, *p0, *x0;
+    const double* poses;
+    const int32_t* pose_of_rid;
+    int basis;
+    double* Bmat;
+    double* bg;
+};
+
+#define PS_BJF_SCRATCH(D) (3 * (D) * (D) + 2 * (D))
+
+template <int D>
+PS_DEV void block_jacobi_factor_wave(int i, int lane, double a_in, double* sc, const BjFactorOut& o)
+{
+    constexpr int DD = D * D;
+    double* A = sc;
+    double* Li = sc + DD;
+    double* sB = sc + 2 * DD;
+    double* sR = sc + 3 * DD;
+    const double* gl = sc + 3 * DD + D;
+    const bool with_g = o.r0 != nullptr;
+    if (with_g && i == 0 && lane == 0) { o.status[ST_PCG_DONE] = 0; o.status[ST_PCG_ITERS] = 0; }
+    const bool act = lane < DD;
+    const int r = act ? lane / D : 0, c = act ? lane % D : 0;
+    if (act) { A[lane] = a_in; Li[lane] = 0.0; }
+    __builtin_amdgcn_wave_barrier();
+    bool ok = true;
+#pragma unroll
+    for (int j = 0; j < D; ++j) {
+        const double d = A[j * D + j];
+        ok = ok && (d > 0.0);
+        const double l = sqrt(d);
+        __builtin_amdgcn_wave_barrier();
+        if (act && c == j && r >= j) A[lane] = (r == j) ? l : A[lane] / l;
+        __builtin_amdgcn_wave_barrier();
+        if (act && r > j && c > j) A[lane] -= A[r * D + j] * A[c * D + j];
+        __builtin_amdgcn_wave_barrier();
+    }
+    if (lane < D) {
+        const int cc = lane;
+        double col[D];
+#pragma unroll
+        for (int rr = 0; rr < D; ++rr) {
+            double v = (rr == cc) ? 1.0 : 0.0;
+#pragma unroll
+            for (int k = 0; k < rr; ++k) v -= (k >= cc) ? A[rr * D + k] * col[k] : 0.0;
+            col[rr] = (rr >= cc) ? v / A[rr * D + rr] : 0.0;
+            Li[rr * D + cc] = col[rr];
+        }
+    }
+    __builtin_amdgcn_wave_barrier();
+    if (!ok && lane == 0) atomicAdd(&o.status[ST_DIAG_FAIL], 1);
+    if (act) o.Linv[(size_t)i * DD + lane] = Li[lane];
+    if (with_g && lane < D) {
+        double v = 0.0;
+#pragma unroll
+        for (int k = 0; k < D; ++k) v += Li[lane * D + k] * gl[k];
+        const size_t oo = (size_t)i * D + lane;
+        o.r0[oo] = v; o.w0[oo] = 0.0; o.s0[oo] = 0.0; o.p0[oo] = 0.0; o.x0[oo] = 0.0;
+        sR[lane] = v;
+    }
+    if (!o.Bmat) return;
+    if (act) {
+        typedef PoseOps<D> G;
+        double v = (r == c) ? 1.0 : 0.0;
+        if (o.basis == 1) {
+            const double* Tp = o.poses + G::W * (size_t)o.pose_of_rid[i];
+            v = 0.0;
+#pragma unroll
+            for (int m2 = 0; m2 < D; ++m2) v += (m2 >= r) ? A[m2 * D + r] * G::adj_mem(Tp, m2, c) : 0.0;
+        }
+        o.Bmat[(size_t)i * DD + lane] = v;
+        sB[lane] = v;
+    }
+    __builtin_amdgcn_wave_barrier();
+    if (with_g && lane < D) {
+        double v = 0.0;
+#pragma unroll
+        for (int a = 0; a < D; ++a) v += sB[a * D + lane] * sR[a];
+        o.bg[(size_t)i * D + lane] = v;
+    }
+}
diff --git a/pyslam_amd/csrc/ps_k_cg_fused.h b/pyslam_amd/csrc/ps_k_cg_fused.h
--- a/pyslam_amd/csrc/ps_k_cg_fused.h
+++ b/pyslam_amd/csrc/ps_k_cg_fused.h
@@ -10,72 +10,15 @@
     double* __restrict__ Bmat, double* __restrict__ bg)
 {
     constexpr int DD = D * D;
-    __shared__ double sA[4][DD], sLi[4][DD], sB[4][DD], sR[4][D];
+    __shared__ double sc[4][PS_BJF_SCRATCH(D)];
     const int wv = threadIdx.x >> 6, lane = threadIdx.x & 63;
     const int i = blockIdx.x * 4 + wv;
-    if (g && blockIdx.x == 0 && threadIdx.x == 0) { status[ST_PCG_DONE] = 0; status[ST_PCG_ITERS] = 0; }
     if (i >= nr) return;
-    const bool act = lane < DD;
-    const int r = act ? lane / D : 0, c = act ? lane % D : 0;
-    double* A = sA[wv];
-    double* Li = sLi[wv];
-    if (act) { A[lane] = S[(size_t)diag_slot[i] * DD + lane]; Li[lane] = 0.0; }
-    __builtin_amdgcn_wave_barrier();
-    bool ok = true;
-#pragma unroll
-    for (int j = 0; j < D; ++j) {
-        const double d = A[j * D + j];
-        ok = ok && (d > 0.0);
-        const double l = sqrt(d);
-        __builtin_amdgcn_wave_barrier();
-        if (act && c == j && r >= j) A[lane] = (r == j) ? l : A[lane] / l;
-        __builtin_amdgcn_wave_barrier();
-        if (act && r > j && c > j) A[lane] -= A[r * D + j] * A[c * D + j];
-        __builtin_amdgcn_wave_barrier();
-    }
-    if (lane < D) {
-        const int cc = lane;
-        double col[D];
-#pragma unroll
-        for (int rr = 0; rr < D; ++rr) {
-            double v = (rr == cc) ? 1.0 : 0.0;
-#pragma unroll
-            for (int k = 0; k < rr; ++k) v -= (k >= cc) ? A[rr * D + k] * col[k] : 0.0;
-            col[rr] = (rr >= cc) ? v / A[rr * D + rr] : 0.0;
-            Li[rr * D + cc] = col[rr];
-        }
-    }
-    __builtin_amdgcn_wave_barrier();
-    if (!ok && lane == 0) atomicAdd(&status[ST_DIAG_FAIL], 1);
-    if (act) Linv[(size_t)i * DD + lane] = Li[lane];
-    if (g && lane < D) {
-        double v = 0.0;
-#pragma unroll
-        for (int k = 0; k < D; ++k) v += Li[lane * D + k] * g[(size_t)i * D + k];
-        const size_t o = (size_t)i * D + lane;
-        r0[o] = v; w0[o] = 0.0; s0[o] = 0.0; p0[o] = 0.0; x0[o] = 0.0;
-        sR[wv][lane] = v;
-    }
-    if (!Bmat) return;
-    if (act) {
-        typedef PoseOps<D> G;
-        double v = (r == c) ? 1.0 : 0.0;
-        if (basis == 1) {
-            const double* Tp = poses + G::W * (size_t)pose_of_rid[i];
-            v = 0.0;
-#pragma unroll
-            for (int m2 = 0; m2 < D; ++m2) v += (m2 >= r) ? A[m2 * D + r] * G::adj_mem(Tp, m2, c) : 0.0;
-        }
-        Bmat[(size_t)i * DD + lane] = v;
-        sB[wv][lane] = v;
-    }
-    __builtin_amdgcn_wave_barrier();
-    if (g && lane < D) {
-        double v = 0.0;
-#pragma unroll
-        for (int a = 0; a < D; ++a) v += sB[wv][a * D + lane] * sR[wv][a];
-        bg[(size_t)i * D + lane] = v;
-    }
+    double a_in = 0.0;
+    if (lane < DD) a_in = S[(size_t)diag_slot[i] * DD + lane];
+    if (g && lane < D) sc[wv][3 * DD + D + lane] = g[(size_t)i * D + lane];
+    const BjFactorOut o{Linv, status, g ? r0 : nullptr, w0, s0, p0, x0, poses, pose_of_rid, basis, Bmat, bg};
+    block_jacobi_factor_wave<D>(i, lane, a_in, sc[wv], o);
 }
 
 template <int D>
diff --git a/pyslam_amd/csrc/ps_k_linearize.h b/pyslam_amd/csrc/ps_k_linearize.h
--- a/pyslam_amd/csrc/ps_k_linearize.h
+++ b/pyslam_amd/csrc/ps_k_linearize.h
@@ -302,7 +302,8 @@
 
 PS_DEV void pose_finalize_wave(int rid, int lane, const int32_t* __restrict__ pitem_ptr,
                                const double* __restrict__ partial, const int32_t* __restrict__ diag_slot,
-                               double lambda, double* __restrict__ S, double* __restrict__ g, double* v )
+                               double lambda, double* __restrict__ S, double* __restrict__ g, double* v ,
+                               double* s_new = nullptr, double* g_new = nullptr)
 {
     if (lane < PS_NPOSE_ACC) {
         double s = 0.0;
@@ -310,15 +311,20 @@
         v[lane] = s;
     }
     __builtin_amdgcn_wave_barrier();
+    double sn = 0.0, gn = 0.0;
     if (lane < 36) {
         const int r = lane / 6, c = lane % 6;
         const int a = r < c ? r : c, b = r < c ? c : r;
         const int idx = a * 6 - (a * (a - 1)) / 2 + (b - a);
         double val = v[idx];
         if (r == c) val += lambda * v[27 + r];
-        S[(size_t)diag_slot[rid] * 36 + lane] += val;
-    }
-    if (lane < 6) g[(size_t)rid * 6 + lane] += v[21 + lane];
+        const size_t o = (size_t)diag_slot[rid] * 36 + lane;
+        sn = S[o] + val;
+        S[o] = sn;
+    }
+    if (lane < 6) { const size_t o = (size_t)rid * 6 + lane; gn = g[o] + v[21 + lane]; g[o] = gn; }
+    if (s_new) *s_new = sn;
+    if (g_new) *g_new = gn;
 }
 
 __global__ __launch_bounds__(64) void k_pose_finalize(
diff --git a/pyslam_amd/csrc/ps_k_schur2.h b/pyslam_amd/csrc/ps_k_schur2.h
--- a/pyslam_amd/csrc/ps_k_schur2.h
+++ b/pyslam_amd/csrc/ps_k_schur2.h
@@ -89,7 +89,8 @@
     int per_xcd, const PairItem* __restrict__ xitems, const int2* __restrict__ pairs, const double* __restrict__ Z,
     double* __restrict__ S, double* __restrict__ Spart, int first, int last,
     int fin_first_block, int fin_nr, const int32_t* __restrict__ pitem_ptr, const double* __restrict__ ppartial,
-    const int32_t* __restrict__ diag_slot, double lambda, double* __restrict__ g)
+    const int32_t* __restrict__ diag_slot, double lambda, double* __restrict__ g,
+    BjFactorOut ride, int fin_lead)
 {
     constexpr int ablate = ABL;
     __shared__ __attribute__((aligned(16))) double sbuf[2 * 4 * PS_SQ_BUF];
@@ -98,14 +99,24 @@
     double* const buf0 = sbuf + wv * PS_SQ_BUF;
     double* const buf1 = buf0 + 4 * PS_SQ_BUF;
     int32_t* const islot = sidx + wv * 256;
-    if ((int)blockIdx.x >= fin_first_block) {
-        const int rid = ((int)blockIdx.x - fin_first_block) * 4 + wv;
-        if (rid < fin_nr) pose_finalize_wave(rid, lane, pitem_ptr, ppartial, diag_slot, lambda, S, g, buf0);
+    const int bid = (int)blockIdx.x - fin_lead;
+    if (bid < 0 || bid >= fin_first_block) {
+        const int rid = (bid < 0 ? (int)blockIdx.x : bid - fin_first_block) * 4 + wv;
+        if (rid < fin_nr) {
+            double sv, gv;
+            pose_finalize_wave(rid, lane, pitem_ptr, ppartial, diag_slot, lambda, S, g, buf0, &sv, &gv);
+            if (ride.Linv) {
+                static_assert(64 + PS_BJF_SCRATCH(6) <= PS_SQ_BUF, "the factor's scratch fits the wave's chunk buffer");
+                double* sc = buf0 + 64;
+                if (lane < 6) sc[3 * 36 + 6 + lane] = gv;
+                block_jacobi_factor_wave<6>(rid, lane, sv, sc, ride);
+            }
+        }
         return;
     }
-    const int local = first + (blockIdx.x >> 3) * 4 + wv;
+    const int local = first + (bid >> 3) * 4 + wv;
     if (local >= last) return;
-    const size_t pos = (size_t)(blockIdx.x & 7) * per_xcd + local;
+    const size_t pos = (size_t)(bid & 7) * per_xcd + local;
     PairItem it = xitems[pos];
     it.slot = __builtin_amdgcn_readfirstlane(it.slot); it.slotT = __builtin_amdgcn_readfirstlane(it.slotT);
     it.start = __builtin_amdgcn_readfirstlane(it.start); it.end = __builtin_amdgcn_readfirstlane(it.end);
diff --git a/pyslam_amd/csrc/ps_kernels.h b/pyslam_amd/csrc/ps_kernels.h
--- a/pyslam_amd/csrc/ps_kernels.h
+++ b/pyslam_amd/csrc/ps_kernels.h
@@ -62,6 +62,7 @@
 }
 
 #include "ps_k_linearize.h"
+#include "ps_k_bjfactor.h"
 #include "ps_k_schur2.h"
 #include "ps_k_pcg_classic.h"
 #include "ps_k_ldi.h"
```
